# henreedev/audio-pathtracer

Measured on NVIDIA B200. Metric: bdpt_path_pairs_per_second, higher is better.
Workload: dtype f32 + u64 Q32.32

## Files before the change

### audio-pathtracer_b200/csrc/fs_api.cu

```cuda
#include "fs_internal.h"

#include <nvtx3/nvToolsExt.h>
#include <stdio.h>
#include <utility>
#include <stdlib.h>
#include <new>
#include <vector>

static thread_local std::string g_err;

#define CK(call)                                                                              \
    do {                                                                                      \
        cudaError_t e__ = (call);                                                             \
        if (e__ != cudaSuccess) return fail_cuda(ctx, e__, #call);                            \
    } while (0)

static int fail(fs_ctx* ctx, int code, const char* msg)
{
    (void)ctx;
    g_err = msg;
    return code;
}
static int fail_cuda(fs_ctx* ctx, cudaError_t e, const char* what)
{
// ... 17 lines not shown
};

extern "C" {

void fs_default_config(fs_config* c)
{
    memset(c, 0, sizeof(*c));
    c->n_bands = 8; c->n_bins = 1000; c->bin_ms = 1.0f; c->rr_prob = 0.9f;
    c->eps_offset = 1e-3f; c->eps_connect = 1e-3f; c->min_seg = 1e-2f; c->sound_speed = 343.0f;
    c->pdf_exponent = 0.1f; c->energy_clamp = 1.0f; c->energy_gain = 10.0f;
    static const float air[FS_MAX_BANDS] = {0.0001f, 0.0003f, 0.0006f, 0.0010f, 0.0017f, 0.0035f, 0.0050f, 0.0120f};
    for (int b = 0; b < FS_MAX_BANDS; ++b) c->air_absorption[b] = air[b];
    c->sample_rate = 48000; c->n_channels = 2; c->ir_threshold = 1e-6f; c->ir_lowpass = 0.25f;
    c->conv_block = 1024; c->conv_clamp = 1; c->conv_wet = 1.0f;
    c->max_batch_paths = 0; c->flags = 0; c->device = -1;
}

const char* fs_last_error(const fs_ctx* ctx) { (void)ctx; return g_err.c_str(); }

int fs_create(const fs_config* cfg, fs_ctx** out)
{
    if (!cfg || !out) return fail(nullptr, FS_ERR_INVALID, "fs_create: null argument");
    *out = nullptr;
    if (cfg->n_bands < 1 || cfg->n_bands > FS_MAX_BANDS) return fail(nullptr, FS_ERR_INVALID, "n_bands must be 1..8");
    if (cfg->n_bins < 1 || cfg->n_bins > (1u << 20)) return fail(nullptr, FS_ERR_INVALID, "n_bins out of range");
    if (!(cfg->bin_ms > 0.f) || !(cfg->sound_speed > 0.f)) return fail(nullptr, FS_ERR_INVALID, "bin_ms/sound_speed must be > 0");
    if (!(cfg->rr_prob > 0.f) || cfg->rr_prob > 1.0f) return fail(nullptr, FS_ERR_INVALID, "rr_prob must be in (0,1]");
    if (cfg->n_channels < 1 || cfg->n_channels > 8) return fail(nullptr, FS_ERR_INVALID, "n_channels must be 1..8");
    if (cfg->conv_block < 32 || cfg->conv_block > 2048 || (cfg->conv_block & (cfg->conv_block - 1)))
        return fail(nullptr, FS_ERR_INVALID, "conv_block must be a power of two in 32..2048");
    if (cfg->sample_rate < cfg->conv_block) return fail(nullptr, FS_ERR_INVALID, "sample_rate < conv_block");
    if ((uint32_t)((double)cfg->bin_ms * 1e-3 * cfg->sample_rate + 0.5) < 1u)
        return fail(nullptr, FS_ERR_INVALID, "bin_ms * sample_rate / 1000 must be at least one sample");
    if (!(cfg->ir_lowpass > 0.0f) || cfg->ir_lowpass > 1.0f) return fail(nullptr, FS_ERR_INVALID, "ir_lowpass must be in (0,1]");
    uint32_t ir_window = 32;
    if (cfg->ir_lowpass < 1.0f) {
        const double w = ceil(log(1e-12) / log(1.0 - (double)cfg->ir_lowpass));
        if (!(w <= 8192.0)) return fail(nullptr, FS_ERR_INVALID, "ir_lowpass too small (needs a warm-up window above 8192 samples)");
        ir_window = ((uint32_t)w + 31u) & ~31u;
        if (ir_window < 32u) ir_window = 32u;
    }
    int ndev = 0;
    cudaError_t e = cudaGetDeviceCount(&ndev);
    if (e != cudaSuccess || ndev == 0) {
        char buf[256];
        snprintf(buf, sizeof(buf), "no usable CUDA device (%s); this library has no CPU fallback",
                 e == cudaSuccess ? "device count 0" : cudaGetErrorString(e));
        return fail(nullptr, FS_ERR_CUDA, buf);
    }
    int dev = cfg->device;
    if (dev < 0) { if (cudaGetDevice(&dev) != cudaSuccess) dev = 0; }
    if (dev >= ndev) return fail(nullptr, FS_ERR_INVALID, "device ordinal out of range");
    fs_ctx* ctx = new (std::nothrow) fs_ctx();
    if (!ctx) return fail(nullptr, FS_ERR_NOMEM, "out of host memory");
    ctx->cfg = *cfg;
    if (ctx->cfg.max_batch_paths == 0) ctx->cfg.max_batch_paths = 1u << 21;
    ctx->device = dev;
    ctx->ir_window = ir_window;
    ctx->launches.store(0); ctx->conv_active.store(0);
    ctx->tune_refill = 4; ctx->tune_leaf_max = FS_LEAF_MAX; ctx->tune_tex = 2; ctx->tune_builder = 1; ctx->tune_wide = 1; ctx->tune_node_min = 14; ctx->tune_tri_min = 4; ctx->tune_collapse = 17 ; ctx->tune_l2pin_mb = 0xffffffffu ; ctx->tune_streams = 2;
    if (const char* e14 = getenv("FS_TUNE_STREAMS")) { int v = atoi(e14); if (v >= 1 && v <= FS_MAX_LANES) ctx->tune_streams = (uint32_t)v; } ctx->tune_tq = 2;
    ctx->tune_tq_node_min = 10; ctx->tune_tq_flush = 24;
    if (const char* e11 = getenv("FS_TUNE_TQ")) ctx->tune_tq = (uint32_t)atoi(e11);
    ctx->tune_mega = 2;
    if (const char* e15 = getenv("FS_TUNE_MEGA")) ctx->tune_mega = (uint32_t)atoi(e15);
    ctx->tune_mega_from = 0; ctx->tune_mega_lanes = 2;
    if (const char* e16 = getenv("FS_TUNE_MEGA_FROM")) ctx->tune_mega_from = (uint32_t)atoi(e16);
    if (const char* e17 = getenv("FS_TUNE_MEGA_LANES")) { int v = atoi(e17); if (v >= 1 && v <= FS_MAX_LANES) ctx->tune_mega_lanes = (uint32_t)v; }
    if (const char* e12 = getenv("FS_TUNE_TQ_NODE_MIN")) ctx->tune_tq_node_min = (uint32_t)atoi(e12);
    if (const char* e13 = getenv("FS_TUNE_TQ_FLUSH")) ctx->tune_tq_flush = (uint32_t)atoi(e13);
    if (ctx->tune_tq_flush < 1) ctx->tune_tq_flush = 1;
    if (ctx->tune_tq_flush > 32) ctx->tune_tq_flush = 32;
    if (const char* e10 = getenv("FS_TUNE_L2PIN")) ctx->tune_l2pin_mb = (uint32_t)atoi(e10);
    if (const char* e9 = getenv("FS_TUNE_COLLAPSE")) ctx->tune_collapse = (uint32_t)atoi(e9);
    if (const char* e7 = getenv("FS_TUNE_TRI_MIN")) ctx->tune_tri_min = (uint32_t)atoi(e7);
    if (const char* e6 = getenv("FS_TUNE_NODE_MIN")) ctx->tune_node_min = (uint32_t)atoi(e6);
    if (const char* e5 = getenv("FS_TUNE_WIDE")) ctx->tune_wide = (uint32_t)atoi(e5);
    ctx->tune_w8 = 0;
    if (const char* e18 = getenv("FS_TUNE_W8")) ctx->tune_w8 = (uint32_t)atoi(e18);
    if (const char* e4 = getenv("FS_TUNE_BUILDER")) ctx->tune_builder = (uint32_t)atoi(e4);
    if (const char* e3 = getenv("FS_TUNE_TEX")) ctx->tune_tex = (uint32_t)atoi(e3);
    if (const char* e1 = getenv("FS_TUNE_REFILL")) { int v = atoi(e1); if (v >= 1 && v <= 32) ctx->tune_refill = (uint32_t)v; }
    if (const char* e2 = getenv("FS_TUNE_LEAF_MAX")) { int v = atoi(e2); if (v >= 1 && v <= 8) ctx->tune_leaf_max = (uint32_t)v; }
    dev_guard g(dev);
    int rc = FS_OK;
    do {
        cudaDeviceProp prop;
        if ((e = cudaGetDeviceProperties(&prop, dev)) != cudaSuccess) { rc = fail_cuda(nullptr, e, "cudaGetDeviceProperties"); break; }
        if (prop.major < 10) {
            char buf[256];
            snprintf(buf, sizeof(buf), "device %d is sm_%d%d; this library is built for sm_100a only", dev, prop.major, prop.minor);
            rc = fail(nullptr, FS_ERR_CUDA, buf); break;
        }
        ctx->sm_count = prop.multiProcessorCount;
        if ((e = cudaStreamCreateWithFlags(&ctx->own_stream, cudaStreamNonBlocking)) != cudaSuccess) { rc = fail_cuda(nullptr, e, "cudaStreamCreate"); break; }
        ctx->stream = ctx->own_stream;
        if ((e = cudaEventCreate(&ctx->ev0)) != cudaSuccess || (e = cudaEventCreate(&ctx->ev1)) != cudaSuccess ||
            (e = cudaEventCreate(&ctx->ev_ir0)) != cudaSuccess || (e = cudaEventCreate(&ctx->ev_ir1)) != cudaSuccess) { rc = fail_cuda(nullptr, e, "cudaEventCreate"); break; }
        if ((e = cudaEventCreateWithFlags(&ctx->ev_fork, cudaEventDisableTiming)) != cudaSuccess) { rc = fail_cuda(nullptr, e, "cudaEventCreate"); break; }
        if ((e = cudaEventCreateWithFlags(&ctx->ev_overflow, cudaEventDisableTiming)) != cudaSuccess) { rc = fail_cuda(nullptr, e, "cudaEventCreate"); break; }
        if ((e = cudaEventCreate(&ctx->ev_c0)) != cudaSuccess || (e = cudaEventCreate(&ctx->ev_c1)) != cudaSuccess) { rc = fail_cuda(nullptr, e, "cudaEventCreate"); break; }
        if ((e = cudaMallocHost(&ctx->h_overflow, sizeof(uint32_t))) != cudaSuccess) { rc = fail_cuda(nullptr, e, "cudaMallocHost"); break; }
        *ctx->h_overflow = 0u;
        for (int l = 1; l < FS_MAX_LANES && e == cudaSuccess; ++l) {
            if ((e = cudaStreamCreateWithFlags(&ctx->lanes[l].stream, cudaStreamNonBlocking)) != cudaSuccess) break;
            e = cudaEventCreateWithFlags(&ctx->lanes[l].done, cudaEventDisableTiming);
        }
        if (e != cudaSuccess) { rc = fail_cuda(nullptr, e, "batch lanes"); break; }
        if ((e = cudaMalloc(&ctx->d_counters, sizeof(fs_dev_counters))) != cudaSuccess) { rc = fail_cuda(nullptr, e, "cudaMalloc counters"); break; }
        if ((e = cudaMemsetAsync(ctx->d_counters, 0, sizeof(fs_dev_counters), ctx->own_stream)) != cudaSuccess ||
            (e = cudaStreamSynchronize(ctx->own_stream)) != cudaSuccess) { rc = fail_cuda(nullptr, e, "cudaMemset"); break; }
        if ((e = cudaMalloc(&ctx->d_amp, sizeof(float) * cfg->n_bins)) != cudaSuccess) { rc = fail_cuda(nullptr, e, "cudaMalloc amp"); break; }
        if ((e = cudaMalloc(&ctx->d_energy, sizeof(float) * cfg->n_bins)) != cudaSuccess) { rc = fail_cuda(nullptr, e, "cudaMalloc energy"); break; }
        if ((e = fs_conv_setup(ctx)) != cudaSuccess) { rc = fail_cuda(nullptr, e, "fs_conv_setup"); break; }
    } while (0);
    if (rc != FS_OK) { fs_destroy(ctx); return rc; }
    *out = ctx;
    return FS_OK;
}

void fs_destroy(fs_ctx* ctx)
{
    if (!ctx) return;
    dev_guard g(ctx->device);
    cudaDeviceSynchronize();
    fs_conv_teardown(ctx);
    cudaFree(ctx->d_carriers); cudaFree(ctx->d_amp_bands); cudaFree(ctx->d_amp_all);
    cudaFree(ctx->lis_rec); cudaFree(ctx->lis_end);
    for (int l = 0; l < FS_MAX_LANES; ++l) {
        fs_wave_free(&ctx->lanes[l].wb);
        if (l && ctx->lanes[l].stream) cudaStreamDestroy(ctx->lanes[l].stream);
        if (ctx->lanes[l].done) cudaEventDestroy(ctx->lanes[l].done);
    }
    if (ctx->ev_fork) cudaEventDestroy(ctx->ev_fork);
    if (ctx->ev_overflow) cudaEventDestroy(ctx->ev_overflow);
    if (ctx->ev_c0) cudaEventDestroy(ctx->ev_c0);
    if (ctx->ev_c1) cudaEventDestroy(ctx->ev_c1);
    if (ctx->h_overflow) cudaFreeHost(ctx->h_overflow);
    cudaFree(ctx->d_bsdf_tab); cudaFree(ctx->d_lobes);
    fs_bvh_free(&ctx->bvh);
    cudaFree(ctx->d_verts); cudaFree(ctx->d_tri_mat); cudaFree(ctx->d_refl_over_pi);
    cudaFree(ctx->d_hist); cudaFree(ctx->d_counters); cudaFree(ctx->d_src_pos); cudaFree(ctx->d_dbg);
    cudaFree(ctx->d_amp); cudaFree(ctx->d_energy);
    for (cudaEvent_t e : ctx->kev) cudaEventDestroy(e);
    for (cudaEvent_t e : ctx->tev) cudaEventDestroy(e);
    if (ctx->ev0) cudaEventDestroy(ctx->ev0);
    if (ctx->ev1) cudaEventDestroy(ctx->ev1);
    if (ctx->ev_ir0) cudaEventDestroy(ctx->ev_ir0);
    if (ctx->ev_ir1) cudaEventDestroy(ctx->ev_ir1);
    if (ctx->own_stream) cudaStreamDestroy(ctx->own_stream);
    delete ctx;
}

static void apply_l2_policy(fs_ctx* ctx);

static int check_overflow(fs_ctx* ctx, bool wait)
{
    if (!ctx->overflow_pending) return FS_OK;
    if (wait) { CK(cudaEventSynchronize(ctx->ev_overflow)); }
    else if (cudaEventQuery(ctx->ev_overflow) != cudaSuccess) { (void)cudaGetLastError(); return FS_OK; }
    ctx->overflow_pending = false;
    if (*ctx->h_overflow) {
        *ctx->h_overflow = 0u;
        return fail(ctx, FS_ERR_OVERFLOW, "BVH traversal stack overflow in the last trace (tree deeper than FS_STACK_SIZE): its histogram is incomplete");
    }
    return FS_OK;
// ... 95 lines not shown
int fs_scene_set_materials_ex(fs_ctx* ctx, const float* absorption, const float* transmission, const float* scattering,
                              const float* thickness_cm, uint32_t n_materials, uint32_t n_bands)
{
    int rc = fs_scene_set_materials(ctx, absorption, n_materials, n_bands);
    if (rc != FS_OK) return rc;
    const size_t n = (size_t)n_materials * n_bands;
    for (int which = 0; which < 2; ++which) {
        const float* v = which ? scattering : transmission;
        if (!v) continue;
        for (size_t i = 0; i < n; ++i)
            if (!(v[i] >= 0.0f && v[i] <= 1.0f)) return fail(ctx, FS_ERR_INVALID, which ? "scattering must be in [0,1]" : "transmission must be in [0,1]");
    }
    if (thickness_cm)
        for (uint32_t m = 0; m < n_materials; ++m)
            if (!(thickness_cm[m] >= 0.0f)) return fail(ctx, FS_ERR_INVALID, "thickness must be >= 0");
    ctx->mat_transmission.assign(transmission ? transmission : nullptr, transmission ? transmission + n : nullptr);
    ctx->mat_scattering.assign(scattering ? scattering : nullptr, scattering ? scattering + n : nullptr);
    ctx->mat_thickness_cm.assign(thickness_cm ? thickness_cm : nullptr, thickness_cm ? thickness_cm + n_materials : nullptr);
    ctx->committed = false;
    return FS_OK;
}

static int build_material_model(fs_ctx* ctx)
{
    const uint32_t M = ctx->n_mats, B = ctx->cfg.n_bands;
    std::vector<float> tab((size_t)3 * M * B, 0.0f);
    std::vector<float4> lobes(M);
    const float* tr = ctx->mat_transmission.empty() ? nullptr : ctx->mat_transmission.data();
    const float* sc = ctx->mat_scattering.empty() ? nullptr : ctx->mat_scattering.data();
    const float* th = ctx->mat_thickness_cm.empty() ? nullptr : ctx->mat_thickness_cm.data();
    for (uint32_t m = 0; m < M; ++m) {
        float sum_r = 0.0f, sum_t = 0.0f, sum_s = 0.0f;
        const float thick = th ? th[m] : 2.5f;
        const float ex = thick / 2.5f;
        for (uint32_t b = 0; b < B; ++b) {
            const float a = ctx->mat_absorption[(size_t)m * B + b];
            const float refl = 1.0f - a;
            float tau = tr ? tr[(size_t)m * B + b] : 0.0f;
            if (refl + tau > 1.0f) tau = 1.0f - refl;
            const float sig = sc ? sc[(size_t)m * B + b] : 1.0f;
            float tau_eff = 0.0f;
            if (tau > 0.0f) tau_eff = (ex == 1.0f) ? tau : fs_pow(tau, ex);
            tab[((size_t)0 * M + m) * B + b] = (refl * sig) / FS_PI;
            tab[((size_t)1 * M + m) * B + b] = refl * (1.0f - sig);
            tab[((size_t)2 * M + m) * B + b] = tau_eff;
            sum_r += refl; sum_t += tau; sum_s += sig;
        }
        const float mr = sum_r / (float)B, mt = sum_t / (float)B, ms = sum_s / (float)B;
        const float tot = mr + mt;
        const float t1 = (tot > 0.0f) ? mt / tot : 0.0f;
        const float ps = (1.0f - t1) * (1.0f - ms);
        const float t2 = t1 + ps;
        const float pd = 1.0f - t2;
        lobes[m] = make_float4(t1, t2, ps, pd);
    }
    cudaFree(ctx->d_bsdf_tab); cudaFree(ctx->d_lobes); ctx->d_bsdf_tab = nullptr; ctx->d_lobes = nullptr;
    CK(cudaMalloc(&ctx->d_bsdf_tab, sizeof(float) * tab.size()));
    CK(cudaMalloc(&ctx->d_lobes, sizeof(float4) * lobes.size()));
    CK(cudaMemcpyAsync(ctx->d_bsdf_tab, tab.data(), sizeof(float) * tab.size(), cudaMemcpyHostToDevice, ctx->stream));
    CK(cudaMemcpyAsync(ctx->d_lobes, lobes.data(), sizeof(float4) * lobes.size(), cudaMemcpyHostToDevice, ctx->stream));
    CK(cudaStreamSynchronize(ctx->stream));
    return FS_OK;
}

int fs_scene_commit(fs_ctx* ctx)
{
    if (!ctx) return FS_ERR_INVALID;
    if (!ctx->tris_set || !ctx->mats_set) return fail(ctx, FS_ERR_STATE, "fs_scene_commit: set triangles and materials first");
    nvtx_range nv("fs_scene_commit (BVH build)");
    dev_guard g(ctx->device);
    if (ctx->n_tris) {
        std::vector<uint32_t> m(ctx->n_tris);
        CK(cudaMemcpyAsync(m.data(), ctx->d_tri_mat, sizeof(uint32_t) * ctx->n_tris, cudaMemcpyDeviceToHost, ctx->stream));
        CK(cudaStreamSynchronize(ctx->stream));
        for (uint64_t i = 0; i < ctx->n_tris; ++i)
            if (m[i] >= ctx->n_mats) return fail(ctx, FS_ERR_INVALID, "triangle material id out of range");
    }
    if (ctx->cfg.flags & FS_FLAG_MATERIAL_MODEL) {
        int rc = build_material_model(ctx);
        if (rc) return rc;
    }
    uint64_t bvh_launches = 0;
    CK(fs_bvh_build(ctx->stream, ctx->d_verts, ctx->d_tri_mat, ctx->n_tris, &ctx->bvh, &bvh_launches,
                    ctx->tune_leaf_max, ctx->tune_builder, ctx->tune_collapse | (ctx->tune_w8 ? 4u : 0u)));
    CK(cudaStreamSynchronize(ctx->stream));
    ctx->launches.fetch_add(bvh_launches);
    ctx->stats.bvh_nodes = ctx->bvh.n_inner;
    if (getenv("FS_VERBOSE")) fprintf(stderr, "[frequensee] BVH: %u triangles, %u BVH2 nodes, %u reachable 4-wide nodes (%.1f MB)\n",
                                      ctx->bvh.n_tris, ctx->bvh.n_inner, ctx->bvh.n_wide, ctx->bvh.n_wide * 64.0 / 1e6);
    if (getenv("FS_VERBOSE") && ctx->bvh.w8nodes) fprintf(stderr, "[frequensee] BVH: %u 8-wide compressed nodes (%.1f MB)\n", ctx->bvh.n_w8, ctx->bvh.n_w8 * 80.0 / 1e6);
    ctx->stats.bvh_max_leaf = ctx->bvh.max_leaf;
    apply_l2_policy(ctx);
    ctx->committed = true;
    ctx->verts_dirty = false;
    return FS_OK;
}

static bool host_is_pinned(const void* p);

int fs_scene_update_vertices(fs_ctx* ctx, const float* verts, uint64_t first_tri, uint64_t n_tris)
{
    if (!ctx) return FS_ERR_INVALID;
    if (!ctx->tris_set) return fail(ctx, FS_ERR_STATE, "fs_scene_update_vertices: call fs_scene_set_triangles first");
    if (n_tris && !verts) return fail(ctx, FS_ERR_INVALID, "fs_scene_update_vertices: null array");
    if (first_tri > ctx->n_tris || n_tris > ctx->n_tris - first_tri)
        return fail(ctx, FS_ERR_INVALID, "fs_scene_update_vertices: triangle range outside the scene");
    for (uint64_t i = 0; i < n_tris * 9; ++i)
        if (!(verts[i] == verts[i]) || fabsf(verts[i]) > 1e18f) return fail(ctx, FS_ERR_INVALID, "non-finite vertex");
    if (!n_tris) return FS_OK;
    dev_guard g(ctx->device);
    CK(cudaMemcpyAsync(ctx->d_verts + first_tri * 9, verts, sizeof(float) * 9 * n_tris, cudaMemcpyHostToDevice, ctx->stream));
    if (host_is_pinned(verts)) CK(cudaStreamSynchronize(ctx->stream));
    if (ctx->committed) ctx->verts_dirty = true;
    return FS_OK;
}

int fs_scene_refit(fs_ctx* ctx, float* cost_ratio_out)
{
    if (!ctx) return FS_ERR_INVALID;
    if (!ctx->committed) return fail(ctx, FS_ERR_STATE, "fs_scene_refit: call fs_scene_commit first");
    nvtx_range nv("fs_scene_refit");
    if (ctx->tune_w8) {
        int rc = fs_scene_commit(ctx);
        if (rc == FS_OK && cost_ratio_out) *cost_ratio_out = 1.0f;
        return rc;
    }
    dev_guard g(ctx->device);
    uint64_t launches = 0;
    float ratio = 1.0f;
    CK(fs_bvh_refit(ctx->stream, ctx->d_verts, &ctx->bvh, &launches, &ratio));
    ctx->launches.fetch_add(launches);
    ctx->verts_dirty = false;
    if (cost_ratio_out) *cost_ratio_out = ratio;
    return FS_OK;
}

static void fill_params(fs_ctx* ctx, fs_trace_params* tp, const float lis[3], uint64_t n_paths, uint32_t max_depth,
                        uint64_t seed)
{
    const fs_config& c = ctx->cfg;
    memset(tp, 0, sizeof(*tp));
    tp->bv.nodes_tex = (ctx->tune_tex && ctx->bvh.nodes_tex) ? (unsigned long long)ctx->bvh.nodes_tex : 0ull;
    tp->bv.tris_tex = (ctx->tune_tex && ctx->bvh.tris_tex) ? (unsigned long long)ctx->bvh.tris_tex : 0ull;
    tp->bv.wnodes = ctx->tune_wide ? ctx->bvh.wnodes : nullptr;
    tp->bv.wnodes_tex = (ctx->tune_tex && ctx->bvh.wnodes_tex) ? (unsigned long long)ctx->bvh.wnodes_tex : 0ull;
    const bool w8 = ctx->tune_w8 && ctx->tune_wide && ctx->bvh.w8nodes;
    tp->bv.w8nodes = w8 ? ctx->bvh.w8nodes : nullptr; tp->bv.tris8 = w8 ? ctx->bvh.tris8 : nullptr; tp->bv.tri8_map = w8 ? ctx->bvh.tri8_map : nullptr;
    tp->bv.w8_magic = 0x47000000u;
    for (int a = 0; a < 3; ++a) { tp->bv.qbase[a] = ctx->bvh.qbase[a]; tp->bv.qscale[a] = ctx->bvh.qscale[a]; }
    tp->bv.nodes = ctx->bvh.nodes; tp->bv.tris = ctx->bvh.tris; tp->bv.tri_orig = ctx->bvh.tri_orig;
    tp->bv.tri_mat = ctx->bvh.tri_mat; tp->bv.tri_nm = ctx->bvh.tri_nm; tp->bv.n_tris = ctx->bvh.n_tris; tp->bv.n_inner = ctx->bvh.n_inner;
    tp->top = ctx->bvh.top_nodes; tp->n_top = ctx->bvh.n_top;
    const bool model = (c.flags & FS_FLAG_MATERIAL_MODEL) && ctx->d_lobes;
    tp->refl_over_pi = model ? ctx->d_bsdf_tab : ctx->d_refl_over_pi; tp->n_mats = ctx->n_mats;
    tp->lobes = model ? ctx->d_lobes : nullptr;
    tp->ep.min_seg = c.min_seg; tp->ep.pdf_exponent = c.pdf_exponent; tp->ep.n_bands = c.n_bands;
    for (int b = 0; b < FS_MAX_BANDS; ++b) tp->ep.air[b] = c.air_absorption[b];
    tp->n_bins = c.n_bins; tp->bin_ms = c.bin_ms; tp->rr_prob = c.rr_prob; tp->eps_offset = c.eps_offset;
    tp->eps_connect = c.eps_connect; tp->sound_speed = c.sound_speed; tp->energy_clamp = c.energy_clamp;
    tp->energy_gain = c.energy_gain; tp->max_depth = max_depth;
    tp->seed_lo = (uint32_t)seed; tp->seed_hi = (uint32_t)(seed >> 32);
    tp->n_paths = n_paths;
    tp->src_pos = ctx->d_src_pos;
    if (lis) { tp->lis[0] = lis[0]; tp->lis[1] = lis[1]; tp->lis[2] = lis[2]; }
    tp->flags = c.flags;
}

// ... 676 lines not shown
```

### audio-pathtracer_b200/csrc/fs_bvh.cuh

```cuda
#pragma once

#include "fs_math.cuh"

#define FS_STACK_SIZE 64
#define FS_LEAF_MAX 4
#define FS_TOP_FLAG 0x40000000

#if defined(FS_TRAVERSAL_GUARD)
#define FS_GUARD_DECL uint32_t guard_ = 0;
#define FS_GUARD_STEP if (++guard_ > 4000000u) { *overflow = 2u; node = SENTINEL; sp = 0; break; }
#else
#define FS_GUARD_DECL
#define FS_GUARD_STEP
#endif

struct fs_bvh_view {
    unsigned long long nodes_tex;
    unsigned long long tris_tex;
    unsigned long long wnodes_tex;
    const uint4* wnodes;
    const uint4* w8nodes;
    const float4* tris8;
    const uint32_t* tri8_map;
    uint32_t w8_magic;
    float qbase[3], qscale[3];
    const float4* nodes;
    const float4* tris;
    const uint32_t* tri_orig;
    const uint32_t* tri_mat;
    const float4* tri_nm;
    uint32_t n_tris;
    uint32_t n_inner;
};

struct fs_visit_counters { uint32_t nodes, tris; };

#if defined(__CUDACC__)

__device__ __forceinline__ float4 fs_ldg4(const float4* p)
{
    float4 r;
    asm volatile("ld.global.nc.v4.f32 {%0, %1, %2, %3}, [%4];"
                 : "=f"(r.x), "=f"(r.y), "=f"(r.z), "=f"(r.w) : "l"(p));
    return r;
}

__device__ __forceinline__ void fs_ldg8(const float4* p, float4& a, float4& b)
{
    asm volatile("ld.global.nc.v8.f32 {%0, %1, %2, %3, %4, %5, %6, %7}, [%8];"
                 : "=f"(a.x), "=f"(a.y), "=f"(a.z), "=f"(a.w), "=f"(b.x), "=f"(b.y), "=f"(b.z), "=f"(b.w)
                 : "l"(p));
}

struct fs_ray_prep {
    fs_vec3 o, d;
    float idx, idy, idz, oodx, oody, oodz;
};

__device__ __forceinline__ fs_ray_prep fs_prep_ray(fs_vec3 o, fs_vec3 d)
{
    fs_ray_prep r;
    r.o = o; r.d = d;
    float dx = (fabsf(d.x) > 1e-30f) ? d.x : ((d.x < 0.0f) ? -1e-30f : 1e-30f);
    float dy = (fabsf(d.y) > 1e-30f) ? d.y : ((d.y < 0.0f) ? -1e-30f : 1e-30f);
    float dz = (fabsf(d.z) > 1e-30f) ? d.z : ((d.z < 0.0f) ? -1e-30f : 1e-30f);
    r.idx = 1.0f / dx; r.idy = 1.0f / dy; r.idz = 1.0f / dz;
    r.oodx = o.x * r.idx; r.oody = o.y * r.idy; r.oodz = o.z * r.idz;
    return r;
}

__device__ __forceinline__ void fs_slab2(const fs_ray_prep& r, float4 n0, float4 n1, float4 n2,
                                         float tmax, bool& h0, bool& h1, float& t0n, float& t1n)
{
    float c0lox = fmaf(n0.x, r.idx, -r.oodx), c0hix = fmaf(n0.y, r.idx, -r.oodx);
    float c0loy = fmaf(n0.z, r.idy, -r.oody), c0hiy = fmaf(n0.w, r.idy, -r.oody);
    float c0loz = fmaf(n2.x, r.idz, -r.oodz), c0hiz = fmaf(n2.y, r.idz, -r.oodz);
    float c1lox = fmaf(n1.x, r.idx, -r.oodx), c1hix = fmaf(n1.y, r.idx, -r.oodx);
    float c1loy = fmaf(n1.z, r.idy, -r.oody), c1hiy = fmaf(n1.w, r.idy, -r.oody);
    float c1loz = fmaf(n2.z, r.idz, -r.oodz), c1hiz = fmaf(n2.w, r.idz, -r.oodz);
    float c0min = fmaxf(fmaxf(fminf(c0lox, c0hix), fminf(c0loy, c0hiy)), fmaxf(fminf(c0loz, c0hiz), 0.0f));
    float c0max = fminf(fminf(fmaxf(c0lox, c0hix), fmaxf(c0loy, c0hiy)), fminf(fmaxf(c0loz, c0hiz), tmax));
    float c1min = fmaxf(fmaxf(fminf(c1lox, c1hix), fminf(c1loy, c1hiy)), fmaxf(fminf(c1loz, c1hiz), 0.0f));
    float c1max = fminf(fminf(fmaxf(c1lox, c1hix), fmaxf(c1loy, c1hiy)), fminf(fmaxf(c1loz, c1hiz), tmax));
    h0 = c0min <= c0max;
    h1 = c1min <= c1max;
    t0n = c0min; t1n = c1min;
}

// ... 117 lines not shown
```

### audio-pathtracer_b200/csrc/fs_bvh_build.cu

```cuda
#include "fs_internal.h"
#include <vector>
#include <utility>
#include <stdlib.h>

namespace {

__device__ __forceinline__ uint32_t f2ord(float f)
{
    uint32_t u = __float_as_uint(f);
    return (u & 0x80000000u) ? ~u : (u | 0x80000000u);
}
__host__ __device__ __forceinline__ float ord2f(uint32_t u)
{
    u = (u & 0x80000000u) ? (u & 0x7fffffffu) : ~u;
#if defined(__CUDA_ARCH__)
    return __uint_as_float(u);
#else
    float f; memcpy(&f, &u, 4); return f;
#endif
}

__global__ void k_init_bounds(uint32_t* bounds)
{
    if (threadIdx.x < 3) bounds[threadIdx.x] = 0xffffffffu;
// ... 469 lines not shown
    cbox c[4];
    int k = 2;
    load_children(nodes, (int)i, c[0], c[1]);
    if (collapse) {
        while (k < 4) {
            int pick = -1; float best = -1.0f;
            for (int j = 0; j < k; ++j)
                if (c[j].ref >= 0) { const float a = cbox_area(c[j]); if (a > best) { best = a; pick = j; } }
            if (pick < 0) break;
            const int r = c[pick].ref;
            load_children(nodes, r, c[pick], c[k]);
            ++k;
        }
    } else {
        const int r0 = c[0].ref, r1 = c[1].ref;
        if (r1 >= 0) { load_children(nodes, r1, c[1], c[k]); ++k; }
        if (r0 >= 0) { load_children(nodes, r0, c[0], c[k]); ++k; }
    }
    for (int j = 0; j < 4; ++j) {
        wnodes[(size_t)i * 4 + j] = (j < k) ? quant_box(c[j].lx, c[j].hx, c[j].ly, c[j].hy, c[j].lz, c[j].hz, c[j].ref, grid) : EMPTY;
        wsrc[(size_t)i * 4 + j] = (j < k) ? c[j].src : -1;
    }
}

__device__ __forceinline__ bool wide_is_inner(uint32_t ref) { return (int)ref >= 0 && ref != 0x7fffffffu; }

__global__ void k_wide_count(const uint4* __restrict__ src, const int* __restrict__ frontier, uint32_t nf, uint32_t* __restrict__ cnt)
{
    const uint32_t t = blockIdx.x * blockDim.x + threadIdx.x;
    if (t >= nf) return;
    const uint4* p = src + (size_t)frontier[t] * 4;
    uint32_t c = 0;
    for (int j = 0; j < 4; ++j) c += wide_is_inner(p[j].w) ? 1u : 0u;
    cnt[t] = c;
}

__global__ void k_wide_place(const uint4* __restrict__ src, uint4* __restrict__ dst, const int* __restrict__ src_prov,
                             int* __restrict__ dst_prov, const int* __restrict__ frontier, uint32_t nf,
                             const uint32_t* __restrict__ off, uint32_t level_base, int* __restrict__ next_frontier)
{
    const uint32_t t = blockIdx.x * blockDim.x + threadIdx.x;
    if (t >= nf) return;
    const uint4* p = src + (size_t)frontier[t] * 4;
    uint4* q = dst + (size_t)(level_base + t) * 4;
    uint32_t o = off[t];
    for (int j = 0; j < 4; ++j) {
        uint4 u = p[j];
        if (wide_is_inner(u.w)) { next_frontier[o] = (int)u.w; u.w = level_base + nf + o; ++o; }
        q[j] = u;
        dst_prov[(size_t)(level_base + t) * 4 + j] = src_prov[(size_t)frontier[t] * 4 + j];
    }
}

#define W8_EMPTY 0x7fffffff
__device__ __forceinline__ uint32_t q8_lo(float v, float p, float inv)
{
    const float q = floorf((v - p) * inv - 0.001953125f);
    return (uint32_t)fminf(fmaxf(q, 0.0f), 255.0f);
}
__device__ __forceinline__ uint32_t q8_hi(float v, float p, float inv)
{
    const float q = ceilf((v - p) * inv + 0.001953125f);
    return (uint32_t)fminf(fmaxf(q, 0.0f), 255.0f);
}
__device__ __forceinline__ int q8_exponent(float ext)
{
    int k = -60;
    if (ext > 1e-18f) { (void)frexpf(ext / 254.0f, &k); }
    k = k < -60 ? -60 : (k > 60 ? 60 : k);
    return k + 127;
}

__global__ void k_w8_parents(uint32_t n_inner, const float4* __restrict__ nodes, int* __restrict__ parent, uint32_t* __restrict__ need)
{
    const uint32_t i = blockIdx.x * blockDim.x + threadIdx.x;
    if (i >= n_inner) return;
    const float4 n3 = nodes[(size_t)i * 4 + 3];
    const int c0 = __float_as_int(n3.x), c1 = __float_as_int(n3.y);
    need[i] = (c0 >= 0 ? 1u : 0u) + (c1 >= 0 ? 1u : 0u);
    if (c0 >= 0) parent[c0] = (int)i;
    if (c1 >= 0) parent[c1] = (int)i;
    if (i == 0) parent[0] = -1;
}
template <int W>
__device__ __forceinline__ float wide_t(const float* T, int ref, int j) { return ref >= 0 ? __ldcg(T + (size_t)ref * W + (j - 1)) : 0.0f; }
__device__ __forceinline__ float w8_t(const float* T, int ref, int j) { return wide_t<8>(T, ref, j); }
template <int W>
__global__ void k_wide_dp(uint32_t n_inner, const float4* __restrict__ nodes, const int* __restrict__ parent,
                        const uint32_t* __restrict__ need, uint32_t* __restrict__ arrive, float* T)
{
    const uint32_t i = blockIdx.x * blockDim.x + threadIdx.x;
    if (i >= n_inner || need[i] != 0u) return;
    int n = (int)i;
    for (;;) {
        cbox a, b;
        load_children(nodes, n, a, b);
        float ta[W], tb[W], t[W];
        for (int j = 1; j <= W; ++j) { ta[j - 1] = wide_t<W>(T, a.ref, j); tb[j - 1] = wide_t<W>(T, b.ref, j); }
        cbox u;
        u.lx = fminf(a.lx, b.lx); u.hx = fmaxf(a.hx, b.hx); u.ly = fminf(a.ly, b.ly); u.hy = fmaxf(a.hy, b.hy);
        u.lz = fminf(a.lz, b.lz); u.hz = fmaxf(a.hz, b.hz);
        float best = 3.0e38f;
        for (int x = 1; x <= W - 1; ++x) best = fminf(best, ta[x - 1] + tb[W - 1 - x]);
        t[0] = cbox_area(u) + best;
        for (int j = 2; j <= W; ++j) {
            float m = t[j - 2];
            for (int x = 1; x < j; ++x) m = fminf(m, ta[x - 1] + tb[j - x - 1]);
            t[j - 1] = m;
        }
        for (int j = 0; j < W; ++j) T[(size_t)n * W + j] = t[j];
        __threadfence();
        const int p = parent[n];
        if (p < 0) break;
        if (atomicAdd(arrive + p, 1u) + 1u < need[p]) break;
        n = p;
    }
}

template <int W>
__device__ __forceinline__ int dp_cut(const float4* __restrict__ nodes, const float* __restrict__ T, int i, cbox* c)
{
    cbox st[W]; int sb[W]; int sp = 0, k = 0;
    {
        cbox l, r;
        load_children(nodes, i, l, r);
        float best = 3.0e38f; int ba = 1;
        for (int x = 1; x <= W - 1; ++x) { const float v = wide_t<W>(T, l.ref, x) + wide_t<W>(T, r.ref, W - x); if (v < best) { best = v; ba = x; } }
        st[0] = l; sb[0] = ba; st[1] = r; sb[1] = W - ba; sp = 2;
    }
    while (sp) {
        --sp;
        const cbox m = st[sp]; const int j = sb[sp];
        if (m.ref < 0 || j == 1) { c[k++] = m; continue; }
        cbox x, y;
        load_children(nodes, m.ref, x, y);
        float best = wide_t<W>(T, m.ref, 1); int ba = 0;
        for (int q = 1; q < j; ++q) { const float v = wide_t<W>(T, x.ref, q) + wide_t<W>(T, y.ref, j - q); if (v < best) { best = v; ba = q; } }
        if (!ba) { c[k++] = m; continue; }
        st[sp] = x; sb[sp] = ba; st[sp + 1] = y; sb[sp + 1] = j - ba; sp += 2;
    }
    return k;
}

__global__ void k_emit4_dp(uint32_t n_inner, const float4* __restrict__ nodes, const float* __restrict__ T, const float* __restrict__ grid,
                           uint4* __restrict__ wnodes, int* __restrict__ wsrc)
{
    const uint32_t i = blockIdx.x * blockDim.x + threadIdx.x;
    if (i >= n_inner) return;
    const uint4 EMPTY = make_uint4(0x0000ffffu, 0x0000ffffu, 0x0000ffffu, 0x7fffffffu);
    cbox c[4];
    const int k = dp_cut<4>(nodes, T, (int)i, c);
    for (int j = 0; j < 4; ++j) {
        wnodes[(size_t)i * 4 + j] = (j < k) ? quant_box(c[j].lx, c[j].hx, c[j].ly, c[j].hy, c[j].lz, c[j].hz, c[j].ref, grid) : EMPTY;
        wsrc[(size_t)i * 4 + j] = (j < k) ? c[j].src : -1;
    }
}

__global__ void k_emit8(uint32_t n_inner, const float4* __restrict__ nodes, const float* __restrict__ T, uint4* __restrict__ w8tmp,
                        int* __restrict__ w8ref)
{
    const uint32_t i = blockIdx.x * blockDim.x + threadIdx.x;
    if (i >= n_inner) return;
    cbox c[8];
    int k = 2;
    if (T) {
        k = dp_cut<8>(nodes, T, (int)i, c);
    } else {
        load_children(nodes, (int)i, c[0], c[1]);
        while (k < 8) {
            int pick = -1; float best = -1.0f;
            for (int j = 0; j < k; ++j)
                if (c[j].ref >= 0) { const float a = cbox_area(c[j]); if (a > best) { best = a; pick = j; } }
            if (pick < 0) break;
            const int r = c[pick].ref;
            load_children(nodes, r, c[pick], c[k]);
            ++k;
        }
    }
    float lx = c[0].lx, hx = c[0].hx, ly = c[0].ly, hy = c[0].hy, lz = c[0].lz, hz = c[0].hz;
    for (int j = 1; j < k; ++j) {
        lx = fminf(lx, c[j].lx); hx = fmaxf(hx, c[j].hx); ly = fminf(ly, c[j].ly); hy = fmaxf(hy, c[j].hy);
        lz = fminf(lz, c[j].lz); hz = fmaxf(hz, c[j].hz);
    }
    if (!(hx < 1e29f) || !(lx > -1e29f) || !(hy < 1e29f) || !(hz < 1e29f)) {
        hx = fminf(hx, 1e29f); hy = fminf(hy, 1e29f); hz = fminf(hz, 1e29f);
    }
    const float mx = 0.5f * (lx + hx), my = 0.5f * (ly + hy), mz = 0.5f * (lz + hz);
    int slot_of[8], child_in[8];
    for (int j = 0; j < 8; ++j) { slot_of[j] = -1; child_in[j] = -1; }
    for (int it = 0; it < k; ++it) {
        float best = -3.0e38f; int bc = -1, bs = -1;
        for (int j = 0; j < k; ++j) {
            if (slot_of[j] >= 0) continue;
            const float dx = 0.5f * (c[j].lx + c[j].hx) - mx, dy = 0.5f * (c[j].ly + c[j].hy) - my, dz = 0.5f * (c[j].lz + c[j].hz) - mz;
            for (int s = 0; s < 8; ++s) {
                if (child_in[s] >= 0) continue;
                const float cost = ((s & 1) ? dx : -dx) + ((s & 2) ? dy : -dy) + ((s & 4) ? dz : -dz);
                if (cost > best) { best = cost; bc = j; bs = s; }
            }
        }
        slot_of[bc] = bs; child_in[bs] = bc;
    }
    const int ebx = q8_exponent(hx - lx), eby = q8_exponent(hy - ly), ebz = q8_exponent(hz - lz);
    const float ix = __uint_as_float((uint32_t)(254 - ebx) << 23), iy = __uint_as_float((uint32_t)(254 - eby) << 23),
                iz = __uint_as_float((uint32_t)(254 - ebz) << 23);
    uint32_t q[12];
    for (int w = 0; w < 12; ++w) q[w] = 0u;
    uint32_t imask = 0, lmask = 0;
    int refs[8];
    for (int s = 0; s < 8; ++s) {
        const int j = child_in[s];
        uint32_t b[6];
        if (j < 0) { b[0] = b[1] = b[2] = 255u; b[3] = b[4] = b[5] = 0u; refs[s] = W8_EMPTY; }
        else {
            b[0] = q8_lo(c[j].lx, lx, ix); b[1] = q8_lo(c[j].ly, ly, iy); b[2] = q8_lo(c[j].lz, lz, iz);
            b[3] = q8_hi(c[j].hx, lx, ix); b[4] = q8_hi(c[j].hy, ly, iy); b[5] = q8_hi(c[j].hz, lz, iz);
            refs[s] = c[j].ref;
            if (c[j].ref >= 0) imask |= 1u << s; else lmask |= 1u << s;
        }
        for (int a = 0; a < 6; ++a) q[a * 2 + (s >> 2)] |= b[a] << (8 * (s & 3));
    }
    uint4* o = w8tmp + (size_t)i * 5;
    o[0] = make_uint4(__float_as_uint(lx), __float_as_uint(ly), __float_as_uint(lz), ((uint32_t)ebx << 23) | imask | (lmask << 8));
    o[1] = make_uint4((uint32_t)eby << 23, (uint32_t)ebz << 23, 0u, 0u);
    o[2] = make_uint4(q[0], q[1], q[2], q[3]);
    o[3] = make_uint4(q[4], q[5], q[6], q[7]);
    o[4] = make_uint4(q[8], q[9], q[10], q[11]);
    for (int s = 0; s < 8; ++s) w8ref[(size_t)i * 8 + s] = refs[s];
}

__global__ void k_w8_count(const uint4* __restrict__ w8tmp, const int* __restrict__ frontier, uint32_t nf,
                           uint32_t* __restrict__ cnt_in, uint32_t* __restrict__ cnt_leaf)
{
    const uint32_t t = blockIdx.x * blockDim.x + threadIdx.x;
    if (t >= nf) return;
    const uint32_t w = w8tmp[(size_t)frontier[t] * 5].w;
    cnt_in[t] = (uint32_t)__popc(w & 0xffu);
    cnt_leaf[t] = (uint32_t)__popc((w >> 8) & 0xffu);
}

__global__ void k_w8_place(const uint4* __restrict__ w8tmp, const int* __restrict__ w8ref, uint4* __restrict__ dst,
                           const int* __restrict__ frontier, uint32_t nf, const uint32_t* __restrict__ off_in,
                           const uint32_t* __restrict__ off_leaf, uint32_t level_base, uint32_t tri_level_base,
                           int* __restrict__ next_frontier, const float4* __restrict__ tris, float4* __restrict__ tris8,
                           uint32_t* __restrict__ tri8_map)
{
    const uint32_t t = blockIdx.x * blockDim.x + threadIdx.x;
    if (t >= nf) return;
    const int src = frontier[t];
// ... 502 lines not shown
    BCHECK(cudaStreamSynchronize(st));
    {
        uint64_t acc = 0;
        for (int bin = 4095; bin >= 0; --bin) {
            acc += h_hist[bin];
            if (acc * 10 >= n_slots) { thr = ord2f((uint32_t)bin << 20); break; }
        }
    }
    prev = cost0;
    for (it = 0; it < iters; ++it) {
        struct { double cost; uint32_t moved; } h;
        BCHECK(cudaMemsetAsync(lock, 0, 8ull * n_inner, st));
        BCHECK(cudaMemsetAsync(misc, 0, 16, st));
        k_w8_parents<<<gi, TPB, 0, st>>>(n_inner, nodes, parent, need);
        k_ri_search<<<gs, TPB, 0, st>>>(n_inner, nodes, parent, thr, 1e-5f, mv_gain, mv_dst);
        k_ri_lock<<<gs, TPB, 0, st>>>(n_inner, parent, mv_gain, mv_dst, lock);
        BCHECK(cudaMemcpyAsync(backup, nodes, sizeof(float4) * 4ull * n_inner, cudaMemcpyDeviceToDevice, st));
        k_ri_apply<<<gs, TPB, 0, st>>>(n_inner, parent, mv_gain, mv_dst, lock, nodes, (uint32_t*)(misc + 8));
        BCHECK(cudaMemsetAsync(arrive, 0, 4ull * n_inner, st));
        k_w8_parents<<<gi, TPB, 0, st>>>(n_inner, nodes, parent, need);
        k_refit_nodes<<<gi, TPB, 0, st>>>(n_inner, d_verts, tri_orig, parent, need, arrive, nodes, ubox);
        k_sah_cost<<<gi, TPB, 0, st>>>(n_inner, nodes, (double*)misc);
        *launches += 7;
        BCHECK(cudaMemcpyAsync(&h, misc, sizeof(h), cudaMemcpyDeviceToHost, st));
        BCHECK(cudaStreamSynchronize(st));
        BCHECK(cudaGetLastError());
        if (h.moved == 0) break;
        if (h.cost > prev) {
            BCHECK(cudaMemcpyAsync(nodes, backup, sizeof(float4) * 4ull * n_inner, cudaMemcpyDeviceToDevice, st));
            BCHECK(cudaStreamSynchronize(st));
            break;
        }
        total_moves += h.moved;
        const bool small = prev - h.cost < 1e-4 * prev;
        prev = h.cost;
        if (small) { ++it; break; }
    }
    if (getenv("FS_VERBOSE"))
        fprintf(stderr, "[frequensee] reinsertion: %d iterations, %u moves, surface-area cost %.6g -> %.6g (%.2f %%)\n", it,
                total_moves, cost0, prev, cost0 > 0.0 ? 100.0 * (prev - cost0) / cost0 : 0.0);
fail:
    cudaFree(parent); cudaFree(need); cudaFree(arrive); cudaFree(ubox); cudaFree(backup); cudaFree(lock);
    cudaFree(mv_gain); cudaFree(mv_dst); cudaFree(hist); cudaFree(misc);
    return err;
}

static cudaError_t wide_compact(cudaStream_t st, uint32_t n_inner, const uint4* sparse, const int* sparse_prov, uint4** dense_out,
                                int** dense_prov_out, uint32_t* n_wide_out, uint64_t* launches)
{
    cudaError_t err = cudaSuccess;
    int* fr[2] = {nullptr, nullptr};
    uint32_t *cnt = nullptr, *off = nullptr, *tile_sums = nullptr, *total = nullptr;
    uint4* dense = nullptr;
    int* dense_prov = nullptr;
    const int TPB = 256;
    uint32_t nf = 1, base = 0;
    int pp = 0;
    const int zero = 0;
    BCHECK(cudaMalloc(&fr[0], 4ull * n_inner)); BCHECK(cudaMalloc(&fr[1], 4ull * n_inner));
    BCHECK(cudaMalloc(&cnt, 4ull * n_inner)); BCHECK(cudaMalloc(&off, 4ull * n_inner));
    BCHECK(cudaMalloc(&tile_sums, 4ull * ((n_inner + SCAN_TILE - 1) / SCAN_TILE + 2)));
    BCHECK(cudaMalloc(&total, 4));
    BCHECK(cudaMalloc(&dense, sizeof(uint4) * 4ull * n_inner));
    BCHECK(cudaMalloc(&dense_prov, sizeof(int) * 4ull * n_inner));
    BCHECK(cudaMemcpyAsync(fr[0], &zero, 4, cudaMemcpyHostToDevice, st));
    while (nf) {
        const uint32_t g = (nf + TPB - 1) / TPB;
        uint32_t next = 0;
        k_wide_count<<<g, TPB, 0, st>>>(sparse, fr[pp], nf, cnt); ++*launches;
        scan_u32(st, cnt, off, nf, tile_sums, total, launches);
        k_wide_place<<<g, TPB, 0, st>>>(sparse, dense, sparse_prov, dense_prov, fr[pp], nf, off, base, fr[pp ^ 1]); ++*launches;
        BCHECK(cudaMemcpyAsync(&next, total, 4, cudaMemcpyDeviceToHost, st));
        BCHECK(cudaStreamSynchronize(st));
        base += nf; nf = next; pp ^= 1;
        if (base + nf > n_inner) { err = cudaErrorUnknown; goto fail; }
    }
    BCHECK(cudaGetLastError());
    *dense_out = dense; dense = nullptr; *dense_prov_out = dense_prov; dense_prov = nullptr; *n_wide_out = base;
fail:
    cudaFree(fr[0]); cudaFree(fr[1]); cudaFree(cnt); cudaFree(off); cudaFree(tile_sums); cudaFree(total); cudaFree(dense); cudaFree(dense_prov);
    return err;
}

static cudaError_t w8_build(cudaStream_t st, uint32_t n, uint32_t n_inner, const float4* nodes, const float4* tris,
                            fs_bvh_device* out, uint64_t* launches, bool dp)
{
    cudaError_t err = cudaSuccess;
    float* T = nullptr; int* parent = nullptr; uint32_t *need = nullptr, *arrive = nullptr;
    uint4 *tmp = nullptr, *dense = nullptr, *fit = nullptr;
    int *ref = nullptr, *fr[2] = {nullptr, nullptr};
    uint32_t *cnt_in = nullptr, *cnt_leaf = nullptr, *off_in = nullptr, *off_leaf = nullptr, *tile_sums = nullptr, *total = nullptr;
    float4* tris8 = nullptr; uint32_t* map = nullptr;
    const int TPB = 256;
    uint32_t nf = 1, base = 0, tri_base = 0;
    int pp = 0;
    const int zero = 0;
    BCHECK(cudaMalloc(&tmp, sizeof(uint4) * 5ull * n_inner));
    BCHECK(cudaMalloc(&ref, 4ull * 8 * n_inner));
    BCHECK(cudaMalloc(&dense, sizeof(uint4) * 5ull * n_inner));
    BCHECK(cudaMalloc(&fr[0], 4ull * n_inner)); BCHECK(cudaMalloc(&fr[1], 4ull * n_inner));
    BCHECK(cudaMalloc(&cnt_in, 4ull * n_inner)); BCHECK(cudaMalloc(&cnt_leaf, 4ull * n_inner));
    BCHECK(cudaMalloc(&off_in, 4ull * n_inner)); BCHECK(cudaMalloc(&off_leaf, 4ull * n_inner));
    BCHECK(cudaMalloc(&tile_sums, 4ull * ((n_inner + SCAN_TILE - 1) / SCAN_TILE + 2)));
    BCHECK(cudaMalloc(&total, 8));
    BCHECK(cudaMalloc(&tris8, sizeof(float4) * 4ull * n));
    BCHECK(cudaMalloc(&map, 4ull * n));
    if (dp) {
        BCHECK(cudaMalloc(&T, sizeof(float) * 8ull * n_inner));
        BCHECK(cudaMalloc(&parent, 4ull * n_inner)); BCHECK(cudaMalloc(&need, 4ull * n_inner)); BCHECK(cudaMalloc(&arrive, 4ull * n_inner));
        BCHECK(cudaMemsetAsync(arrive, 0, 4ull * n_inner, st));
        k_w8_parents<<<(n_inner + TPB - 1) / TPB, TPB, 0, st>>>(n_inner, nodes, parent, need);
        k_wide_dp<8><<<(n_inner + TPB - 1) / TPB, TPB, 0, st>>>(n_inner, nodes, parent, need, arrive, T);
        *launches += 2;
    }
    k_emit8<<<(n_inner + TPB - 1) / TPB, TPB, 0, st>>>(n_inner, nodes, T, tmp, ref); ++*launches;
    BCHECK(cudaMemcpyAsync(fr[0], &zero, 4, cudaMemcpyHostToDevice, st));
    while (nf) {
        const uint32_t g = (nf + TPB - 1) / TPB;
        uint32_t next[2] = {0, 0};
        k_w8_count<<<g, TPB, 0, st>>>(tmp, fr[pp], nf, cnt_in, cnt_leaf); ++*launches;
        scan_u32(st, cnt_in, off_in, nf, tile_sums, total, launches);
        scan_u32(st, cnt_leaf, off_leaf, nf, tile_sums, total + 1, launches);
        k_w8_place<<<g, TPB, 0, st>>>(tmp, ref, dense, fr[pp], nf, off_in, off_leaf, base, tri_base, fr[pp ^ 1], tris, tris8, map);
        ++*launches;
        BCHECK(cudaMemcpyAsync(next, total, 8, cudaMemcpyDeviceToHost, st));
        BCHECK(cudaStreamSynchronize(st));
        base += nf; nf = next[0]; tri_base += next[1]; pp ^= 1;
        if ((uint64_t)base + nf > n_inner || tri_base > n) { err = cudaErrorUnknown; goto fail; }
    }
    BCHECK(cudaGetLastError());
    if (tri_base != n) { err = cudaErrorUnknown; goto fail; }
    BCHECK(cudaMalloc(&fit, sizeof(uint4) * 5ull * base));
    BCHECK(cudaMemcpyAsync(fit, dense, sizeof(uint4) * 5ull * base, cudaMemcpyDeviceToDevice, st));
    BCHECK(cudaStreamSynchronize(st));
    out->w8nodes = fit; fit = nullptr; out->n_w8 = base;
    out->tris8 = tris8; tris8 = nullptr; out->tri8_map = map; map = nullptr;
fail:
    cudaFree(T); cudaFree(parent); cudaFree(need); cudaFree(arrive);
    cudaFree(tmp); cudaFree(ref); cudaFree(dense); cudaFree(fit); cudaFree(fr[0]); cudaFree(fr[1]); cudaFree(cnt_in); cudaFree(cnt_leaf);
    cudaFree(off_in); cudaFree(off_leaf); cudaFree(tile_sums); cudaFree(total); cudaFree(tris8); cudaFree(map);
    return err;
}

cudaError_t fs_bvh_build(cudaStream_t st, const float* d_verts, const uint32_t* d_mats, uint64_t T64,
                         fs_bvh_device* out, uint64_t* launches, uint32_t leaf_max_u, uint32_t builder, uint32_t collapse_u)
{
    const int leaf_max = (int)(leaf_max_u < 1 ? 1 : (leaf_max_u > 8 ? 8 : leaf_max_u));
    const int collapse = (int)collapse_u;
    cudaError_t err = cudaSuccess;
    const uint32_t n = (uint32_t)T64;
    fs_bvh_free(out);
    out->n_tris = n;
    if (n == 0) return cudaSuccess;
    const uint32_t n_inner = n > 1 ? n - 1 : 1;
    const uint32_t n_blocks_sort = (n + SORT_TILE - 1) / SORT_TILE;
    float4 *tlo = nullptr, *thi = nullptr, *bb_lo = nullptr, *bb_hi = nullptr;
    uint64_t *keys0 = nullptr, *keys1 = nullptr;
    uint32_t *vals0 = nullptr, *vals1 = nullptr, *block_hist = nullptr, *misc = nullptr, *arrive = nullptr;
    float* grid = nullptr;
    int2 *children = nullptr, *ranges = nullptr;
    int *parent = nullptr, *queue = nullptr;
    const int TPB = 256;
    const uint32_t gb = (n + TPB - 1) / TPB;

    BCHECK(cudaMalloc(&tlo, sizeof(float4) * n));
    BCHECK(cudaMalloc(&thi, sizeof(float4) * n));
    BCHECK(cudaMalloc(&bb_lo, sizeof(float4) * (2ull * n)));
    BCHECK(cudaMalloc(&bb_hi, sizeof(float4) * (2ull * n)));
    BCHECK(cudaMalloc(&keys0, 8ull * n));
    BCHECK(cudaMalloc(&keys1, 8ull * n));
    BCHECK(cudaMalloc(&vals0, 4ull * n));
    BCHECK(cudaMalloc(&vals1, 4ull * n));
    BCHECK(cudaMalloc(&block_hist, 4ull * 256 * n_blocks_sort));
    BCHECK(cudaMalloc(&misc, 4 * 16));
    BCHECK(cudaMalloc(&arrive, 4ull * n_inner));
    BCHECK(cudaMalloc(&children, sizeof(int2) * n_inner));
    BCHECK(cudaMalloc(&ranges, sizeof(int2) * n_inner));
    BCHECK(cudaMalloc(&parent, 4ull * 2 * n));
    BCHECK(cudaMalloc(&queue, 4ull * FS_TOP_CAP));
    BCHECK(cudaMalloc(&out->nodes, sizeof(float4) * 4ull * n_inner));
    BCHECK(cudaMalloc(&out->wnodes, sizeof(uint4) * 4ull * n_inner));
    BCHECK(cudaMalloc(&out->wsrc, sizeof(int) * 4ull * n_inner));
    BCHECK(cudaMalloc(&grid, sizeof(float) * 8));
    BCHECK(cudaMalloc(&out->tris, sizeof(float4) * 4ull * n));
    BCHECK(cudaMalloc(&out->tri_orig, 4ull * n));
    BCHECK(cudaMalloc(&out->tri_mat, 4ull * n));
    BCHECK(cudaMalloc(&out->tri_nm, sizeof(float4) * (size_t)n));
    BCHECK(cudaMalloc(&out->top_nodes, sizeof(float4) * 4ull * FS_TOP_CAP));
    out->n_inner = n_inner;

    BCHECK(cudaMemsetAsync(misc, 0, 4 * 16, st));
    BCHECK(cudaMemsetAsync(arrive, 0, 4ull * n_inner, st));
    k_init_bounds<<<1, 32, 0, st>>>(misc); ++*launches;
    k_tri_bounds<<<gb, TPB, 0, st>>>(d_verts, n, tlo, thi, misc, misc + 6); ++*launches;
    k_morton<<<gb, TPB, 0, st>>>(tlo, thi, n, misc, keys0, vals0); ++*launches;
    {
        uint64_t *ki = keys0, *ko = keys1;
        uint32_t *vi = vals0, *vo = vals1;
        for (int pass = 0; pass < 8; ++pass) {
            int shift = pass * 8;
            k_sort_hist<<<n_blocks_sort, SORT_THREADS, 0, st>>>(ki, n, shift, block_hist, n_blocks_sort);
            k_sort_scan<<<1, 1024, 0, st>>>(block_hist, 256u * n_blocks_sort);
            k_sort_scatter<<<n_blocks_sort, SORT_THREADS, 0, st>>>(ki, vi, ko, vo, n, shift, block_hist, n_blocks_sort);
            *launches += 3;
            uint64_t* tk = ki; ki = ko; ko = tk;
            uint32_t* tv = vi; vi = vo; vo = tv;
        }
    }
    k_pack<<<gb, TPB, 0, st>>>(d_verts, d_mats, vals0, n, tlo, thi, out->tris, out->tri_orig, out->tri_mat, out->tri_nm, bb_lo, bb_hi);
    ++*launches;
    if (n == 1) {
        k_emit_single<<<1, 1, 0, st>>>(bb_lo, bb_hi, out->nodes); ++*launches;
        out->max_leaf = 1;
    } else if (builder == 1 && n >= 3) {
        int cand[4] = {5, 10, 24, 64}, n_cand = 4;
        if (const char* e = getenv("FS_TUNE_PLOC_R")) { int v = atoi(e); if (v >= 1 && v <= 256) { cand[0] = v; n_cand = 1; } }
        if (n < 4096) n_cand = 1;
        double best_cost = 0.0; int best = -1;
        float4* alt = nullptr; double* d_cost = nullptr;
        float* cT4 = nullptr; int* cpar = nullptr; uint32_t *cneed = nullptr, *carr = nullptr;
        if (n_cand > 1) { BCHECK(cudaMalloc(&alt, sizeof(float4) * 4ull * n_inner)); BCHECK(cudaMalloc(&d_cost, 8)); }
        for (int ci = 0; ci < n_cand; ++ci) {
            float4* dst = (n_cand > 1) ? alt : out->nodes;
            BCHECK(ploc_build(st, n, bb_lo, bb_hi, dst, launches, cand[ci]));
            if (n_cand == 1) break;
            double h_cost = 0.0;
            BCHECK(cudaMemsetAsync(d_cost, 0, 8, st));
            k_sah_cost<<<(n_inner + TPB - 1) / TPB, TPB, 0, st>>>(n_inner, dst, d_cost); ++*launches;
            BCHECK(cudaMemcpyAsync(&h_cost, d_cost, 8, cudaMemcpyDeviceToHost, st));
            BCHECK(cudaStreamSynchronize(st));
            if (getenv("FS_VERBOSE")) fprintf(stderr, "[frequensee] PLOC radius %d: surface-area cost %.6g\n", cand[ci], h_cost);
            if (collapse & 16) {
                if (!cT4) {
                    BCHECK(cudaMalloc(&cT4, sizeof(float) * 4ull * n_inner)); BCHECK(cudaMalloc(&cpar, 4ull * n_inner));
                    BCHECK(cudaMalloc(&cneed, 4ull * n_inner)); BCHECK(cudaMalloc(&carr, 4ull * n_inner));
                }
                float root_cost = 0.f;
                BCHECK(cudaMemsetAsync(carr, 0, 4ull * n_inner, st));
                k_w8_parents<<<(n_inner + TPB - 1) / TPB, TPB, 0, st>>>(n_inner, dst, cpar, cneed);
                k_wide_dp<4><<<(n_inner + TPB - 1) / TPB, TPB, 0, st>>>(n_inner, dst, cpar, cneed, carr, cT4);
                *launches += 2;
                BCHECK(cudaMemcpyAsync(&root_cost, cT4, 4, cudaMemcpyDeviceToHost, st));
                BCHECK(cudaStreamSynchronize(st));
                if (getenv("FS_VERBOSE")) fprintf(stderr, "[frequensee] PLOC radius %d: summed area of the 4-wide nodes %.6g\n", cand[ci], (double)root_cost);
                h_cost = (double)root_cost;
            }
            if (best < 0 || h_cost < best_cost) {
                best = ci; best_cost = h_cost;
                BCHECK(cudaMemcpyAsync(out->nodes, alt, sizeof(float4) * 4ull * n_inner, cudaMemcpyDeviceToDevice, st));
            }
        }
        if (alt) { cudaStreamSynchronize(st); cudaFree(alt); cudaFree(d_cost); }
        cudaFree(cT4); cudaFree(cpar); cudaFree(cneed); cudaFree(carr);
        out->max_leaf = 1;
        {
            int sweeps = 0;
            if (const char* e = getenv("FS_TUNE_ROTATE")) { int v = atoi(e); if (v >= 0 && v <= 64) sweeps = v; }
            if (sweeps && n >= 4096) {
                uint32_t n_rot = 0;
                BCHECK(bvh2_rotate(st, n_inner, out->nodes, sweeps, launches, &n_rot));
                if (getenv("FS_VERBOSE")) {
                    double* d_c = nullptr; double h_c = 0.0;
                    if (cudaMalloc(&d_c, 8) == cudaSuccess) {
                        cudaMemsetAsync(d_c, 0, 8, st);
                        k_sah_cost<<<(n_inner + TPB - 1) / TPB, TPB, 0, st>>>(n_inner, out->nodes, d_c);
                        cudaMemcpyAsync(&h_c, d_c, 8, cudaMemcpyDeviceToHost, st); cudaStreamSynchronize(st); cudaFree(d_c);
                    }
                    fprintf(stderr, "[frequensee] %d rotation sweeps: %u rotations, surface-area cost %.6g\n", sweeps, n_rot, h_c);
                }
            }
        }
        {
            int iters = FS_REINSERT_ITERS;
            if (const char* e = getenv("FS_TUNE_REINSERT")) { int v = atoi(e); if (v >= 0 && v <= 256) iters = v; }
            if (iters && n >= 4096) BCHECK(bvh2_reinsert(st, n_inner, d_verts, out->tri_orig, out->nodes, iters, launches));
        }
    } else {
        k_karras<<<gb, TPB, 0, st>>>(keys0, (int)n, children, ranges, parent); ++*launches;
        k_refit<<<gb, TPB, 0, st>>>((int)n, children, parent, bb_lo, bb_hi, arrive); ++*launches;
        k_emit<<<gb, TPB, 0, st>>>((int)n, children, ranges, bb_lo, bb_hi, out->nodes, leaf_max); ++*launches;
        k_leaf_stats<<<gb, TPB, 0, st>>>((int)n, ranges, misc + 8, leaf_max); ++*launches;
    }
    k_quant_grid<<<1, 32, 0, st>>>(out->nodes, grid); ++*launches;
    if ((collapse & 16) && n >= 3) {
        float* T4 = nullptr; int* par = nullptr; uint32_t *need = nullptr, *arr = nullptr;
        cudaError_t e4 = cudaSuccess;
        if ((e4 = cudaMalloc(&T4, sizeof(float) * 4ull * n_inner)) == cudaSuccess && (e4 = cudaMalloc(&par, 4ull * n_inner)) == cudaSuccess &&
            (e4 = cudaMalloc(&need, 4ull * n_inner)) == cudaSuccess && (e4 = cudaMalloc(&arr, 4ull * n_inner)) == cudaSuccess &&
            (e4 = cudaMemsetAsync(arr, 0, 4ull * n_inner, st)) == cudaSuccess) {
            k_w8_parents<<<(n_inner + TPB - 1) / TPB, TPB, 0, st>>>(n_inner, out->nodes, par, need);
            k_wide_dp<4><<<(n_inner + TPB - 1) / TPB, TPB, 0, st>>>(n_inner, out->nodes, par, need, arr, T4);
            k_emit4_dp<<<(n_inner + TPB - 1) / TPB, TPB, 0, st>>>(n_inner, out->nodes, T4, grid, out->wnodes, out->wsrc);
            *launches += 3;
            e4 = cudaStreamSynchronize(st);
        }
        cudaFree(T4); cudaFree(par); cudaFree(need); cudaFree(arr);
        BCHECK(e4);
    } else {
        k_emit4<<<(n_inner + TPB - 1) / TPB, TPB, 0, st>>>(n_inner, out->nodes, grid, out->wnodes, out->wsrc, collapse & 1); ++*launches;
    }
    out->n_wide = n_inner;
    if (!(collapse & 2)) {
        uint4* dense = nullptr; int* dense_prov = nullptr; uint32_t n_wide = 0;
        BCHECK(wide_compact(st, n_inner, out->wnodes, out->wsrc, &dense, &dense_prov, &n_wide, launches));
        cudaFree(out->wnodes); out->wnodes = dense; out->n_wide = n_wide;
        cudaFree(out->wsrc); out->wsrc = dense_prov;
    }
    {
        cudaResourceDesc rd; memset(&rd, 0, sizeof(rd));
        rd.resType = cudaResourceTypeLinear;
        rd.res.linear.devPtr = out->nodes;
        rd.res.linear.desc = cudaCreateChannelDesc<float4>();
        rd.res.linear.sizeInBytes = sizeof(float4) * 4ull * n_inner;
        cudaTextureDesc td; memset(&td, 0, sizeof(td));
        td.readMode = cudaReadModeElementType;
        if (cudaCreateTextureObject(&out->nodes_tex, &rd, &td, nullptr) != cudaSuccess) { out->nodes_tex = 0; (void)cudaGetLastError(); }
        rd.res.linear.devPtr = out->tris;
        rd.res.linear.sizeInBytes = sizeof(float4) * 4ull * n;
        if (cudaCreateTextureObject(&out->tris_tex, &rd, &td, nullptr) != cudaSuccess) { out->tris_tex = 0; (void)cudaGetLastError(); }
        rd.res.linear.devPtr = out->wnodes;
        rd.res.linear.desc = cudaCreateChannelDesc<uint4>();
        rd.res.linear.sizeInBytes = sizeof(uint4) * 4ull * out->n_wide;
        if (cudaCreateTextureObject(&out->wnodes_tex, &rd, &td, nullptr) != cudaSuccess) { out->wnodes_tex = 0; (void)cudaGetLastError(); }
    }
    k_top_treelet<<<1, 32, 0, st>>>(out->nodes, n_inner, FS_TOP_CAP, out->top_nodes, misc + 7, queue); ++*launches;
    BCHECK(cudaGetLastError());
    if (builder == 1 && n >= 3 && out->max_leaf == 1 && (collapse & 4)) BCHECK(w8_build(st, n, n_inner, out->nodes, out->tris, out, launches, !(collapse & 8)));
    {
        uint32_t h[16];
        BCHECK(cudaMemcpyAsync(h, misc, sizeof(h), cudaMemcpyDeviceToHost, st));
        BCHECK(cudaStreamSynchronize(st));
        out->n_top = h[7];
        if (n > 1 && !(builder == 1 && n >= 3)) out->max_leaf = h[8] ? h[8] : 1;
        out->extent = ord2f(h[6]);
        float hg[6];
        BCHECK(cudaMemcpy(hg, grid, sizeof(hg), cudaMemcpyDeviceToHost));
        for (int a = 0; a < 3; ++a) { out->qbase[a] = hg[a]; out->qscale[a] = hg[3 + a]; }
    }
fail:
    cudaFree(tlo); cudaFree(thi); cudaFree(bb_lo); cudaFree(bb_hi); cudaFree(keys0); cudaFree(keys1);
    cudaFree(vals0); cudaFree(vals1); cudaFree(block_hist); cudaFree(misc); cudaFree(arrive);
    cudaFree(children); cudaFree(ranges); cudaFree(parent); cudaFree(queue); cudaFree(grid);
    if (err != cudaSuccess) fs_bvh_free(out);
    return err;
}

void fs_bvh_free(fs_bvh_device* b)
{
    if (b->nodes_tex) cudaDestroyTextureObject(b->nodes_tex);
    if (b->tris_tex) cudaDestroyTextureObject(b->tris_tex);
    if (b->wnodes_tex) cudaDestroyTextureObject(b->wnodes_tex);
    cudaFree(b->w8nodes); cudaFree(b->tris8); cudaFree(b->tri8_map);
    cudaFree(b->nodes); cudaFree(b->wnodes); cudaFree(b->tris); cudaFree(b->tri_orig); cudaFree(b->tri_mat); cudaFree(b->tri_nm); cudaFree(b->top_nodes);
    cudaFree(b->wsrc);
    cudaFree(b->rf.parent); cudaFree(b->rf.need); cudaFree(b->rf.arrive); cudaFree(b->rf.ubox); cudaFree(b->rf.queue); cudaFree(b->rf.misc);
    memset(b, 0, sizeof(*b));
}

cudaError_t fs_bvh_refit(cudaStream_t st, const float* d_verts, fs_bvh_device* b, uint64_t* launches, float* cost_ratio)
{
    cudaError_t err = cudaSuccess;
    const uint32_t n = b->n_tris, n_inner = b->n_inner;
    const int TPB = 256;
    fs_bvh_device::refit_scratch& r = b->rf;
    struct { double cost[2]; float grid[8]; uint32_t n_top; } h;
    if (cost_ratio) *cost_ratio = 1.0f;
    if (n == 0) return cudaSuccess;
    if (!r.misc) {
        BCHECK(cudaMalloc(&r.parent, 4ull * n_inner));
        BCHECK(cudaMalloc(&r.need, 4ull * n_inner));
        BCHECK(cudaMalloc(&r.arrive, 4ull * n_inner));
        BCHECK(cudaMalloc(&r.ubox, sizeof(float4) * 2ull * n_inner));
        BCHECK(cudaMalloc(&r.queue, 4ull * FS_TOP_CAP));
        BCHECK(cudaMalloc(&r.misc, sizeof(h)));
        BCHECK(cudaMemsetAsync(r.parent, 0xff, 4ull * n_inner, st));
        BCHECK(cudaMemsetAsync(r.misc, 0, sizeof(h), st));
        k_w8_parents<<<(n_inner + TPB - 1) / TPB, TPB, 0, st>>>(n_inner, b->nodes, r.parent, r.need);
        k_sah_cost<<<(n_inner + TPB - 1) / TPB, TPB, 0, st>>>(n_inner, b->nodes, (double*)r.misc);
        *launches += 2;
        BCHECK(cudaMemcpyAsync(&r.cost0, r.misc, sizeof(double), cudaMemcpyDeviceToHost, st));
    }
    BCHECK(cudaMemsetAsync(r.arrive, 0, 4ull * n_inner, st));
    BCHECK(cudaMemsetAsync((double*)r.misc + 1, 0, sizeof(double), st));
    k_refit_tris<<<(n + TPB - 1) / TPB, TPB, 0, st>>>(n, d_verts, b->tri_orig, b->tri_mat, b->tris, b->tri_nm);
    if (n == 1) k_refit_single<<<1, 1, 0, st>>>(d_verts, b->tri_orig, b->nodes);
    else k_refit_nodes<<<(n_inner + TPB - 1) / TPB, TPB, 0, st>>>(n_inner, d_verts, b->tri_orig, r.parent, r.need, r.arrive, b->nodes, r.ubox);
    k_sah_cost<<<(n_inner + TPB - 1) / TPB, TPB, 0, st>>>(n_inner, b->nodes, (double*)r.misc + 1);
    {
        float* d_grid = (float*)((char*)r.misc + offsetof(decltype(h), grid));
        k_quant_grid<<<1, 32, 0, st>>>(b->nodes, d_grid);
        const uint32_t n_slots = 4u * b->n_wide;
        k_requant4<<<(n_slots + TPB - 1) / TPB, TPB, 0, st>>>(n_slots, b->nodes, b->wsrc, d_grid, b->wnodes);
        k_top_treelet<<<1, 32, 0, st>>>(b->nodes, n_inner, FS_TOP_CAP, b->top_nodes,
                                        (uint32_t*)((char*)r.misc + offsetof(decltype(h), n_top)), r.queue);
    }
    *launches += 6;
    BCHECK(cudaGetLastError());
    BCHECK(cudaMemcpyAsync(&h, r.misc, sizeof(h), cudaMemcpyDeviceToHost, st));
    BCHECK(cudaStreamSynchronize(st));
    for (int a = 0; a < 3; ++a) { b->qbase[a] = h.grid[a]; b->qscale[a] = h.grid[3 + a]; }
    b->n_top = h.n_top;
    if (cost_ratio) *cost_ratio = r.cost0 > 0.0 ? (float)(h.cost[1] / r.cost0) : 1.0f;
fail:
    return err;
}
```

### audio-pathtracer_b200/csrc/fs_internal.h

```cpp
#pragma once

#include <cuda_runtime.h>
#include <stdint.h>
#include <string.h>
#include <string>
#include <atomic>
#include <mutex>
#include <vector>

#include "../../include/frequensee.h"
#include "fs_math.cuh"
#include "fs_bvh.cuh"

#define FS_TOP_CAP 1024

struct fs_bvh_device {
    float4* nodes;
    float4* tris;
    uint32_t* tri_orig;
    uint32_t* tri_mat;
    float4* tri_nm;
    float4* top_nodes;
    cudaTextureObject_t nodes_tex, tris_tex, wnodes_tex;
    uint4* wnodes;
    float qbase[3], qscale[3];
    uint32_t n_tris, n_inner, n_top, max_leaf;
    uint32_t n_wide;
    uint4* w8nodes;
    float4* tris8;
    uint32_t* tri8_map;
    uint32_t n_w8;
    float extent;
    int* wsrc;
    struct refit_scratch {
        int* parent;
        uint32_t* need;
        uint32_t* arrive;
        float4* ubox;
        int* queue;
        void* misc;
        double cost0;
    } rf;
};

cudaError_t fs_bvh_build(cudaStream_t st, const float* d_verts, const uint32_t* d_mats, uint64_t n_tris,
                         fs_bvh_device* out, uint64_t* launches, uint32_t leaf_max, uint32_t builder ,
                         uint32_t collapse );
void fs_bvh_free(fs_bvh_device* b);
cudaError_t fs_bvh_refit(cudaStream_t st, const float* d_verts, fs_bvh_device* b, uint64_t* launches, float* cost_ratio);

struct fs_dev_counters {
    unsigned long long ext_rays, shadow_rays, connected, node_visits, tri_tests;
    unsigned long long shadow_node_visits, shadow_tri_tests;
    uint32_t overflow, max_steps;
    uint32_t steps_hist[16];
};

struct fs_trace_params {
    fs_bvh_view bv;
    const float4* top;
    uint32_t n_top;
    const float* refl_over_pi;
    const float4* lobes;
    uint32_t n_mats;
    fs_eval_params ep;
    uint32_t n_bins;
    float bin_ms, rr_prob, eps_offset, eps_connect, sound_speed, energy_clamp, energy_gain;
    uint32_t max_depth;
    uint32_t seed_lo, seed_hi;
    uint64_t n_paths;
    uint64_t g_first;
    uint32_t batch;
    uint32_t cap;
    const float* src_pos;
    float lis[3];
    uint32_t flags;
    uint32_t lis_mode;
    float4* lis_rec;
    float4* lis_end;
};

struct fs_wave_buffers {
    float4* st_pos[2];
    float4* st_nrm[2];
    float4* rec;
    float4* end_pos;
    float2* hit;
    uint32_t* conn_queue;
    float* conn_len;
    uint32_t* q_count;
    uint32_t* q_cursor;
    uint32_t cap, depth_cap;
    float4* npos;
    float4* nnrm;
    float4 *all_o, *all_d;
    uint32_t* all_conn;
    uint64_t all_cap;
    float4 *log_o, *log_d; uint32_t* log_flag; void* pq; uint32_t log_cap, pq_epoch;
};

struct fs_conv_source {
    bool active;
    float2* fdl;
    float2* H[2];
    float* prev;
    float* ir;
    int pub, pending;
    cudaEvent_t h_ready[2];
    uint32_t head;
};

#define FS_MEGA_MIN_BATCH (1u << 17)
#define FS_MAX_LANES 4
#define FS_MAX_SOURCES 4096
#define FS_PTR_TABLE 64
struct fs_ptr_table { void* p[FS_PTR_TABLE]; void* q[FS_PTR_TABLE]; };

struct fs_lane { cudaStream_t stream; fs_wave_buffers wb; cudaEvent_t done; };

struct fs_ctx {
    fs_config cfg;
    int device;
    cudaStream_t own_stream, stream;
    cudaStream_t conv_stream;
    float* d_verts; uint32_t* d_tri_mat; uint64_t n_tris;
    float* d_refl_over_pi; uint32_t n_mats;
    float* d_bsdf_tab; float4* d_lobes;
    std::vector<float> mat_absorption;
    std::vector<float> mat_transmission, mat_scattering, mat_thickness_cm;
    bool mats_set, tris_set, committed;
    bool verts_dirty;
    fs_bvh_device bvh;
    fs_lane lanes[FS_MAX_LANES];
    cudaEvent_t ev_fork; uint32_t tune_streams;
    float4 *lis_rec, *lis_end; uint64_t lis_cache_n; uint32_t lis_cache_depth;
    unsigned long long* d_hist; uint32_t hist_sources;
    uint32_t hist_cur_sources;
    uint64_t hist_n_paths;
    fs_dev_counters* d_counters;
    uint32_t* h_overflow; cudaEvent_t ev_overflow; bool overflow_pending;
    float* d_src_pos; uint32_t src_cap;
    fs_path_dbg* d_dbg; uint64_t dbg_cap;
    fs_stats stats;
    std::atomic<uint64_t> launches;
    std::atomic<int> conv_active;
    cudaEvent_t ev0, ev1, ev_ir0, ev_ir1; bool timed, ir_timed;
    std::vector<cudaEvent_t> kev; size_t kev_used;
    std::vector<cudaEvent_t> tev; size_t tev_used;
    int sm_count;
    int occ[16];
    uint32_t tune_refill, tune_leaf_max, tune_tex, tune_builder, tune_wide, tune_node_min, tune_tri_min, tune_collapse, tune_l2pin_mb, tune_tq, tune_tq_node_min, tune_tq_flush, tune_mega, tune_mega_from, tune_mega_lanes, cur_lanes, tune_w8;
    float* d_energy;
    float* d_amp;
    float* d_amp_all; uint32_t amp_all_cap;
    float* d_carriers; float* d_amp_bands; uint64_t carrier_seed;
    float2* d_twiddle;
    uint32_t fft_n, n_part, n_freq, ir_window;
    std::vector<fs_conv_source*> conv;
    float *d_conv_in, *d_conv_out; size_t conv_io_cap;
    float *h_pin_in, *h_pin_out;
    cudaEvent_t ev_c0, ev_c1; float last_conv_ms;
    float* h_pin_ir; size_t pin_ir_cap;
    std::mutex conv_mu;
};

cudaError_t fs_wave_alloc(fs_ctx* ctx, fs_lane* lane, uint32_t cap, uint32_t max_depth);
void fs_wave_free(fs_wave_buffers* wb);
cudaError_t fs_wave_trace_batch(fs_ctx* ctx, fs_lane* lane, const fs_trace_params& tp, unsigned long long* d_hist,
                                fs_path_dbg* d_dbg);
cudaError_t fs_wave_reset_counters(fs_ctx* ctx, int reset_overflow);
cudaError_t fs_wave_debug_rays(fs_ctx* ctx, const fs_trace_params& tp, const float* d_rays, const float* d_tmax,
                               uint64_t n, float* d_t, uint32_t* d_tri, uint8_t* d_hit);

cudaError_t fs_ir_build_multi(fs_ctx* ctx, const unsigned long long* d_hist, uint32_t s0, uint32_t n, uint64_t n_paths,
                              const fs_ptr_table& d_ir);
cudaError_t fs_conv_update_ir_multi(fs_ctx* ctx, uint32_t s0, uint32_t n, cudaStream_t st);
cudaError_t fs_ir_build_bands(fs_ctx* ctx, const unsigned long long* d_hist_src, uint64_t n_paths, uint64_t noise_seed,
                              float* d_ir_out);
cudaError_t fs_ir_build(fs_ctx* ctx, const unsigned long long* d_hist_src, uint64_t n_paths,
                        const float* d_energy_in, float* d_ir_out);

cudaError_t fs_conv_setup(fs_ctx* ctx);
void fs_conv_teardown(fs_ctx* ctx);
cudaError_t fs_conv_source_alloc(fs_ctx* ctx, uint32_t source, bool reset_history);
void fs_conv_source_free(fs_ctx* ctx, uint32_t source);
cudaError_t fs_conv_update_ir(fs_ctx* ctx, uint32_t source, cudaStream_t st);
cudaError_t fs_conv_run(fs_ctx* ctx, const uint32_t* sources, uint32_t n_src, const float* d_in, float* d_out, uint32_t n_blocks,
                        cudaStream_t st);
cudaError_t fs_conv_rfft(fs_ctx* ctx, const float* d_in, uint32_t n, float2* d_out, cudaStream_t st);
```

### audio-pathtracer_b200/csrc/fs_wavefront.cu

```cuda
#include "fs_internal.h"

namespace {

constexpr int WF_THREADS = 256;

#ifndef FS_STREAM_HINTS
#define FS_STREAM_HINTS 0
#endif
#if FS_STREAM_HINTS
#define FS_ST4(ptr, v) __stcs((ptr), (v))
#define FS_ST2(ptr, v) __stcs((ptr), (v))
#define FS_LD4(ptr) __ldcs(ptr)
#define FS_LD2(ptr) __ldcs(ptr)
#else
#define FS_ST4(ptr, v) (*(ptr) = (v))
#define FS_ST2(ptr, v) (*(ptr) = (v))
#define FS_LD4(ptr) (*(ptr))
#define FS_LD2(ptr) (*(ptr))
#endif

enum { MODE_BVH = 0, MODE_TOP = 1, MODE_BRUTE = 2 };

__device__ __forceinline__ uint32_t lane_id() { return threadIdx.x & 31u; }

// ... 965 lines not shown
        }
    }
    (void)guard;
    if (COUNT) flush_counters(dc, vc);
}


#ifndef FS_W8_SSTACK
#define FS_W8_SSTACK 6
#endif
#define FS_W8_STACK_SIZE 40
struct w8_stack {
    uint2* sh;
    uint2* loc;
    __device__ __forceinline__ void put(int i, uint2 e) const { if (i < FS_W8_SSTACK) sh[i * TR_THREADS] = e; else loc[i - FS_W8_SSTACK] = e; }
    __device__ __forceinline__ uint2 get(int i) const { return (i < FS_W8_SSTACK) ? sh[i * TR_THREADS] : loc[i - FS_W8_SSTACK]; }
};

__device__ __forceinline__ void tr_init8(tr_state& s, const fs_bvh_view& bv, fs_vec3 o, fs_vec3 d)
{
    s.o = o; s.d = d;
    const float dx = (fabsf(d.x) > 1e-30f) ? d.x : ((d.x < 0.0f) ? -1e-30f : 1e-30f);
    const float dy = (fabsf(d.y) > 1e-30f) ? d.y : ((d.y < 0.0f) ? -1e-30f : 1e-30f);
    const float dz = (fabsf(d.z) > 1e-30f) ? d.z : ((d.z < 0.0f) ? -1e-30f : 1e-30f);
    s.idx = fs_rcp_fast(dx); s.idy = fs_rcp_fast(dy); s.idz = fs_rcp_fast(dz);
    s.oodx = s.oody = s.oodz = 0.0f;
    s.oct = ((~__float_as_uint(s.idx)) >> 31) | (((~__float_as_uint(s.idy)) >> 31) << 1) | (((~__float_as_uint(s.idz)) >> 31) << 2);
    s.node = bv.n_tris ? 0 : TR_SENT; s.leaf = 0; s.sp = 0; s.tc = 0; s.te = 0;
}

#define FS_Q8(w, B) __uint_as_float(__byte_perm((w), magic, 0x7504u | ((B) << 4)))

__device__ __forceinline__ void w8_step(const fs_bvh_view& bv, tr_state& s, const w8_stack& stack, const float tlimit,
                                        uint32_t& hleaf, uint32_t& lmask, uint32_t& tri_base, uint32_t* overflow)
{
    const uint32_t magic = bv.w8_magic;
    const uint4* p = bv.w8nodes + (size_t)s.node * 5;
    const uint4 u0 = ldg_u4(p), u1 = ldg_u4(p + 1), u2 = ldg_u4(p + 2), u3 = ldg_u4(p + 3), u4 = ldg_u4(p + 4);
    const float ax = __uint_as_float(u0.w & 0x7f800000u) * s.idx, ay = __uint_as_float(u1.x) * s.idy, az = __uint_as_float(u1.y) * s.idz;
    const float bx = fmaf(-32768.0f, ax, (__uint_as_float(u0.x) - s.o.x) * s.idx);
    const float by = fmaf(-32768.0f, ay, (__uint_as_float(u0.y) - s.o.y) * s.idy);
    const float bz = fmaf(-32768.0f, az, (__uint_as_float(u0.z) - s.o.z) * s.idz);
    const bool px = (s.oct & 1u) != 0u, py = (s.oct & 2u) != 0u, pz = (s.oct & 4u) != 0u;
    const uint32_t nx0 = px ? u2.x : u3.z, nx1 = px ? u2.y : u3.w, fx0 = px ? u3.z : u2.x, fx1 = px ? u3.w : u2.y;
    const uint32_t ny0 = py ? u2.z : u4.x, ny1 = py ? u2.w : u4.y, fy0 = py ? u4.x : u2.z, fy1 = py ? u4.y : u2.w;
    const uint32_t nz0 = pz ? u3.x : u4.z, nz1 = pz ? u3.y : u4.w, fz0 = pz ? u4.z : u3.x, fz1 = pz ? u4.w : u3.y;
    uint32_t H = 0u;
#define FS_W8_CHILD(J, W, B)                                                                                          \
    {                                                                                                                 \
        const float tn = fmaxf(fmaxf(fmaf(FS_Q8(nx##W, B), ax, bx), fmaf(FS_Q8(ny##W, B), ay, by)),                   \
                               fmaxf(fmaf(FS_Q8(nz##W, B), az, bz), 0.0f));                                           \
        const float tf = fminf(fminf(fmaf(FS_Q8(fx##W, B), ax, bx), fmaf(FS_Q8(fy##W, B), ay, by)),                   \
                               fminf(fmaf(FS_Q8(fz##W, B), az, bz), tlimit));                                         \
        if (tn <= tf) H |= 1u << (J);                                                                                 \
    }
    FS_W8_CHILD(0, 0, 0u) FS_W8_CHILD(1, 0, 1u) FS_W8_CHILD(2, 0, 2u) FS_W8_CHILD(3, 0, 3u)
    FS_W8_CHILD(4, 1, 0u) FS_W8_CHILD(5, 1, 1u) FS_W8_CHILD(6, 1, 2u) FS_W8_CHILD(7, 1, 3u)
#undef FS_W8_CHILD
    const uint32_t imask = u0.w & 0xffu;
    lmask = (u0.w >> 8) & 0xffu;
    hleaf = H & lmask;
    tri_base = u1.w;
    uint32_t P = H & imask;
    if (s.oct & 4u) P = ((P & 0x0fu) << 4) | (P >> 4);
    if (s.oct & 2u) P = ((P & 0x33u) << 2) | ((P >> 2) & 0x33u);
    if (s.oct & 1u) P = ((P & 0x55u) << 1) | ((P >> 1) & 0x55u);
    uint32_t gb = u1.z, gm = (P << 8) | imask;
    if (P == 0u) {
        if (s.sp == 0) { s.node = TR_SENT; return; }
        --s.sp;
        const uint2 e = stack.get(s.sp);
        gb = e.x; gm = e.y;
    }
    const uint32_t pbit = 31u - (uint32_t)__clz((int)gm);
    gm ^= 1u << pbit;
    const uint32_t slot = (pbit - 8u) ^ s.oct;
    s.node = (int)(gb + (uint32_t)__popc(gm & ((1u << slot) - 1u)));
    if (gm >> 8) {
        if (s.sp < FS_W8_STACK_SIZE) { stack.put(s.sp, make_uint2(gb, gm)); ++s.sp; } else *overflow = 1u;
    }
}

#define FS_TQ_CAP 160
#define TQ_INVALID 0xffffffffu
#define TQ_WARPS (TR_THREADS / 32)
#define TR_SMEM_TQ (FS_SSTACK * TR_THREADS * sizeof(int) + TR_THREADS * sizeof(unsigned long long) + \
                    TQ_WARPS * FS_TQ_CAP * sizeof(uint32_t) + TQ_WARPS * sizeof(uint32_t) + TR_THREADS * sizeof(uint32_t))

#ifndef FS_DRAIN_SPLIT
#define FS_DRAIN_SPLIT 1
#endif
#ifndef FS_PREFETCH_PUSHED
#define FS_PREFETCH_PUSHED 0
#endif
#ifndef FS_PREFETCH_TRIS
#define FS_PREFETCH_TRIS 0
#endif
#ifndef FS_TRI_TEX
#define FS_TRI_TEX 0
#endif
#define FS_TQ8_CAP 288
#define TR_SMEM_TQ8 (FS_W8_SSTACK * TR_THREADS * sizeof(uint2) + TR_THREADS * sizeof(unsigned long long) + \
                     TQ_WARPS * FS_TQ8_CAP * sizeof(uint32_t) + TQ_WARPS * sizeof(uint32_t) + TR_THREADS * sizeof(uint32_t))
template <bool COUNT, int TEX, bool ANY, bool W8>
__global__ void __launch_bounds__(TR_THREADS, FS_TR_MINBLOCKS)
k_trace_q(const fs_bvh_view bv, const float4* __restrict__ ray_o, const float4* __restrict__ ray_d,
          const uint32_t* __restrict__ count_ptr, uint32_t* __restrict__ cursor,
          float2* __restrict__ hits, uint32_t* __restrict__ conn_queue, uint32_t* __restrict__ conn_count,
          fs_path_dbg* __restrict__ dbg, fs_dev_counters* __restrict__ dc, const uint32_t REFILL_MIN,
          const uint32_t NODE_MIN, const uint32_t FLUSH_MIN)
{
    constexpr bool DRAIN_SPLIT = FS_DRAIN_SPLIT != 0;
    constexpr uint32_t QCAP = W8 ? FS_TQ8_CAP : FS_TQ_CAP;
    constexpr int SST = W8 ? FS_W8_SSTACK : FS_SSTACK;
    const uint32_t lane = lane_id(), warp = threadIdx.x >> 5;
    const uint32_t count = *count_ptr;
    extern __shared__ __align__(8) unsigned char smem_raw[];
    int* const sstack = reinterpret_cast<int*>(smem_raw);
    uint2* const gstack = reinterpret_cast<uint2*>(smem_raw);
    unsigned long long* const skey = reinterpret_cast<unsigned long long*>(smem_raw + (W8 ? FS_W8_SSTACK * sizeof(uint2) : FS_SSTACK * sizeof(int)) * TR_THREADS);
    uint32_t* const squeue = reinterpret_cast<uint32_t*>(skey + TR_THREADS) + warp * QCAP;
    uint32_t* const sqcount = reinterpret_cast<uint32_t*>(skey + TR_THREADS) + TQ_WARPS * QCAP + warp;
    uint32_t* const whelp = reinterpret_cast<uint32_t*>(skey + TR_THREADS) + TQ_WARPS * QCAP + TQ_WARPS + (threadIdx.x & ~31u);
    unsigned long long* const mykey = skey + threadIdx.x;
    unsigned long long* const wkey = skey + (threadIdx.x & ~31u);
    int lstack[W8 ? 1 : FS_STACK_SIZE - FS_SSTACK];
    uint2 lstack8[W8 ? FS_W8_STACK_SIZE - FS_W8_SSTACK : 1];
    tr_stack<false> stack; stack.sh = sstack + threadIdx.x; stack.loc = lstack;
    w8_stack stack8; stack8.sh = gstack + threadIdx.x; stack8.loc = lstack8;
    const float4* const tris = W8 ? bv.tris8 : bv.tris;
    const unsigned long long KEY_NONE = ((unsigned long long)0x7f800000u << 32) | 0xffffffffull;
    for (uint32_t i = lane; i < QCAP; i += 32) squeue[i] = TQ_INVALID;
    if (lane == 0) *sqcount = 0u;
    *mykey = KEY_NONE;
    whelp[lane] = 0u;
    uint32_t owner = lane;
    __syncwarp();
    tr_state s;
    s.node = TR_SENT; s.leaf = 0; s.sp = 0; s.tc = 0; s.te = 0;
    s.o = fs_mk(0.f, 0.f, 0.f); s.d = s.o; s.idx = s.idy = s.idz = s.oodx = s.oody = s.oodz = 0.f;
    bool running = false, exhausted = false;
    uint32_t j = 0;
    uint32_t* const ovf_p = &dc->overflow;
    float bt = __int_as_float(0x7f800000);
    uint32_t qn = 0;
    uint32_t ray_steps = 0;
    fs_visit_counters vc; vc.nodes = 0; vc.tris = 0;
    for (;;) {
        const uint32_t m_idle = __ballot_sync(FULLM, !running);
        if (!exhausted && ((uint32_t)__popc(m_idle) >= REFILL_MIN)) {
            const uint32_t n = (uint32_t)__popc(m_idle);
            uint32_t base = 0;
            if (lane == 0) base = atomicAdd(cursor, n);
            base = __shfl_sync(FULLM, base, 0);
            if (base + n >= count) exhausted = true;
            if (!running) {
                const uint32_t jj = base + (uint32_t)__popc(m_idle & ((1u << lane) - 1u));
                if (jj < count) {
                    const float4 a = FS_LD4(ray_o + jj), b = FS_LD4(ray_d + jj);
                    if (W8) tr_init8(s, bv, fs_mk(a.x, a.y, a.z), fs_mk(b.x, b.y, b.z));
                    else tr_init<true>(s, bv, fs_mk(a.x, a.y, a.z), fs_mk(b.x, b.y, b.z));
                    bt = ANY ? a.w : __int_as_float(0x7f800000); *mykey = KEY_NONE;
                    j = ANY ? __float_as_uint(b.w) : jj; running = true;
                    if (COUNT) ray_steps = 0;
                }
            }
        }
        if (!__any_sync(FULLM, running)) break;
        for (;;) {
            for (;;) {
                const bool can = running && s.node >= 0 && s.node != TR_SENT;
                const uint32_t m_can = __ballot_sync(FULLM, can);
                if (m_can == 0u || qn >= FLUSH_MIN) break;
                if (NODE_MIN && qn && (uint32_t)__popc(m_can) < NODE_MIN) break;
                uint32_t nl = 0;
                if (can) {
                    if (COUNT) { vc.nodes++; ray_steps++; }
                    if (W8) {
                        uint32_t hleaf, lmask, tri_base;
                        w8_step(bv, s, stack8, bt, hleaf, lmask, tri_base, ovf_p);
                        nl = (uint32_t)__popc(hleaf);
                        if (nl) {
                            uint32_t* q = squeue + atomicAdd(sqcount, nl);
                            const uint32_t e0 = (tri_base << 5) | owner;
                            do {
                                const uint32_t bit = hleaf & (0u - hleaf);
                                *q++ = e0 + ((uint32_t)__popc(lmask & (bit - 1u)) << 5);
                                hleaf ^= bit;
                            } while (hleaf);
                        }
                    } else {
                        const float INF = __int_as_float(0x7f800000);
                        float k0, k1, k2, k3; int v0, v1, v2, v3;
                        wide_children<2, TEX>(bv, s, bt, k0, k1, k2, k3, v0, v1, v2, v3);
                        const bool l0 = k0 != INF && v0 < 0, l1 = k1 != INF && v1 < 0, l2 = k2 != INF && v2 < 0, l3 = k3 != INF && v3 < 0;
                        nl = (uint32_t)l0 + (uint32_t)l1 + (uint32_t)l2 + (uint32_t)l3;
                        if (nl) {
                            uint32_t* q = squeue + atomicAdd(sqcount, nl);
                            const uint32_t lm4 = owner - 4u;
#if FS_PREFETCH_TRIS
#define FS_PF_TRI(v) asm volatile("prefetch.global.L2 [%0];" :: "l"(bv.tris + (size_t)((uint32_t)(~(v)) >> 3) * 4))
#else
#define FS_PF_TRI(v)
#endif
                            if (l0) { *q = (uint32_t)v0 * 0xfffffffcu + lm4; FS_PF_TRI(v0); }
                            q += l0;
                            if (l1) { *q = (uint32_t)v1 * 0xfffffffcu + lm4; FS_PF_TRI(v1); }
                            q += l1;
                            if (l2) { *q = (uint32_t)v2 * 0xfffffffcu + lm4; FS_PF_TRI(v2); }
                            q += l2;
                            if (l3) { *q = (uint32_t)v3 * 0xfffffffcu + lm4; FS_PF_TRI(v3); }
#undef FS_PF_TRI
                        }
                        k0 = l0 ? INF : k0; k1 = l1 ? INF : k1; k2 = l2 ? INF : k2; k3 = l3 ? INF : k3;
                        FS_CSWAP(k0, v0, k1, v1) FS_CSWAP(k2, v2, k3, v3) FS_CSWAP(k0, v0, k2, v2) FS_CSWAP(k1, v1, k3, v3) FS_CSWAP(k1, v1, k2, v2)
                        w4_advance(s, stack, k0, k1, k2, k3, v0, v1, v2, v3, ovf_p);
                    }
                }
                qn += __reduce_add_sync(FULLM, nl);
            }
            __syncwarp();
            const uint32_t total = qn;
            for (uint32_t base = 0; base < total; base += 32) {
                const uint32_t idx = base + lane;
                const uint32_t e = idx < total ? squeue[idx] : TQ_INVALID;
                const uint32_t eo = e & 31u;
                const float ox = __shfl_sync(FULLM, s.o.x, eo), oy = __shfl_sync(FULLM, s.o.y, eo), oz = __shfl_sync(FULLM, s.o.z, eo);
                const float dx = __shfl_sync(FULLM, s.d.x, eo), dy = __shfl_sync(FULLM, s.d.y, eo), dz = __shfl_sync(FULLM, s.d.z, eo);
                const float bto = __shfl_sync(FULLM, bt, eo);
                if (e != TQ_INVALID) {
                    const uint32_t tri = e >> 5;
                    const float4* tq = tris + (size_t)tri * 4;
#if FS_TRI_TEX
                    const bool ttex = TEX >= 2 && bv.tris_tex;
                    const float4 a = ttex ? tex1Dfetch<float4>((cudaTextureObject_t)bv.tris_tex, (int)(tri * 4u)) : fs_ldg4(tq);
                    const float4 b = (FS_TRI_TEX >= 2 && ttex) ? tex1Dfetch<float4>((cudaTextureObject_t)bv.tris_tex, (int)(tri * 4u + 1u)) : fs_ldg4(tq + 1);
                    const float4 c = fs_ldg4(tq + 2);
#else
                    const float4 a = fs_ldg4(tq), b = fs_ldg4(tq + 1), c = fs_ldg4(tq + 2);
#endif
                    if (COUNT) vc.tris++;
                    squeue[idx] = TQ_INVALID;
                    float t;
                    const bool hit = fs_intersect_tri(fs_mk(ox, oy, oz), fs_mk(dx, dy, dz), fs_mk(a.x, a.y, a.z), fs_mk(b.x, b.y, b.z),
                                                      fs_mk(c.x, c.y, c.z), t);
                    if (ANY) {
                        if (hit && t < bto) *(volatile unsigned long long*)(wkey + eo) = 0ull;
                    } else if (hit && t <= bto) {
                        const unsigned long long mine = ((unsigned long long)__float_as_uint(t) << 32) | tri;
                        unsigned long long old = *(volatile unsigned long long*)(wkey + eo);
                        for (;;) {
                            const float told = __uint_as_float((uint32_t)(old >> 32));
                            bool better = t < told;
                            if (t == told) {
                                const uint32_t otri = (uint32_t)old;
                                better = otri == 0xffffffffu ||
                                         __float_as_uint(fs_ldg4(tq + 3).x) < __float_as_uint(fs_ldg4(tris + (size_t)otri * 4 + 3).x);
                            }
                            if (!better) break;
                            const unsigned long long prev = atomicCAS(wkey + eo, old, mine);
                            if (prev == old) break;
                            old = prev;
                        }
                    }
                }
            }
            __syncwarp();
            if (lane == 0) *sqcount = 0u;
            qn = 0u;
            const unsigned long long kk = *(volatile unsigned long long*)(wkey + owner);
            if (ANY) { if (running && kk != KEY_NONE) { s.node = TR_SENT; s.sp = 0; } }
            else bt = __uint_as_float((uint32_t)(kk >> 32));
            __syncwarp();
            const bool fin = running && s.node == TR_SENT;
            if (fin && owner != lane) { atomicSub(whelp + owner, 1u); running = false; owner = lane; }
            __syncwarp();
            const bool retire = fin && running && *(volatile uint32_t*)(whelp + lane) == 0u;
            if (ANY) {
                const bool conn = retire && kk == KEY_NONE;
                const uint32_t mc = __ballot_sync(FULLM, conn);
                if (mc) {
                    uint32_t slot = 0;
                    if (lane == 0) slot = atomicAdd(conn_count, (uint32_t)__popc(mc));
                    slot = __shfl_sync(FULLM, slot, 0);
                    if (conn) {
                        conn_queue[slot + (uint32_t)__popc(mc & ((1u << lane) - 1u))] = j;
                        if (dbg) dbg[j].connected = 1u;
                    }
                }
                if (retire) running = false;
            } else if (retire) {
                uint32_t ht = (uint32_t)kk;
                if (W8 && ht != 0xffffffffu) ht = bv.tri8_map[ht];
                FS_ST2(hits + j, make_float2(bt, __int_as_float((int)ht)));
                running = false;
                if (COUNT) { atomicMax(&dc->max_steps, ray_steps); atomicAdd(&dc->steps_hist[ray_steps / 8u < 15u ? ray_steps / 8u : 15u], 1u); }
            }
            if (DRAIN_SPLIT && exhausted) {
                const uint32_t m_free = __ballot_sync(FULLM, !running);
                const bool give = running && s.node != TR_SENT && s.sp >= 1 && s.sp <= SST;
                const uint32_t m_give = __ballot_sync(FULLM, give);
                const uint32_t nf = (uint32_t)__popc(m_free), ng = (uint32_t)__popc(m_give);
                const uint32_t n = nf < ng ? nf : ng;
                if (n) {
                    const uint32_t lt = (1u << lane) - 1u;
                    const uint32_t rf = (uint32_t)__popc(m_free & lt), rg = (uint32_t)__popc(m_give & lt);
                    const bool take = !running && rf < n;
                    const uint32_t donor = take ? __fns(m_give, 0u, (int)rf + 1) : lane;
                    const int dsp = __shfl_sync(FULLM, s.sp, donor);
                    const float ox = __shfl_sync(FULLM, s.o.x, donor), oy = __shfl_sync(FULLM, s.o.y, donor), oz = __shfl_sync(FULLM, s.o.z, donor);
                    const float dx = __shfl_sync(FULLM, s.d.x, donor), dy = __shfl_sync(FULLM, s.d.y, donor), dz = __shfl_sync(FULLM, s.d.z, donor);
                    const float ix = __shfl_sync(FULLM, s.idx, donor), iy = __shfl_sync(FULLM, s.idy, donor), iz = __shfl_sync(FULLM, s.idz, donor);
                    const float px = __shfl_sync(FULLM, s.oodx, donor), py = __shfl_sync(FULLM, s.oody, donor), pz = __shfl_sync(FULLM, s.oodz, donor);
                    const float dbt = __shfl_sync(FULLM, bt, donor);
                    const uint32_t down = __shfl_sync(FULLM, owner, donor);
                    if (take) {
                        const int h = (dsp + 1) >> 1;
                        s.o = fs_mk(ox, oy, oz); s.d = fs_mk(dx, dy, dz);
                        s.idx = ix; s.idy = iy; s.idz = iz; s.oodx = px; s.oody = py; s.oodz = pz;
                        bt = dbt; owner = down;
                        if (W8) {
                            const uint2* src = gstack + (threadIdx.x & ~31u) + donor;
                            for (int i = 0; i < h; ++i) stack8.sh[i * TR_THREADS] = src[(dsp - h + i) * TR_THREADS];
                            s.oct = ((~__float_as_uint(ix)) >> 31) | (((~__float_as_uint(iy)) >> 31) << 1) | (((~__float_as_uint(iz)) >> 31) << 2);
                            s.sp = h - 1;
                            const uint2 e = stack8.sh[s.sp * TR_THREADS];
                            uint32_t gm = e.y;
                            const uint32_t pbit = 31u - (uint32_t)__clz((int)gm);
                            gm ^= 1u << pbit;
                            const uint32_t slot = (pbit - 8u) ^ s.oct;
                            s.node = (int)(e.x + (uint32_t)__popc(gm & ((1u << slot) - 1u)));
                            if (gm >> 8) { stack8.sh[s.sp * TR_THREADS] = make_uint2(e.x, gm); ++s.sp; }
                        } else {
                            const int* src = sstack + (threadIdx.x & ~31u) + donor;
                            for (int i = 0; i < h; ++i) stack.sh[i * TR_THREADS] = src[(dsp - h + i) * TR_THREADS];
                            s.sp = h;
                            s.node = stack.pop(s.sp, 0.f);
                        }
                        running = true;
                        atomicAdd(whelp + down, 1u);
                    }
                    __syncwarp();
                    if (give && rg < n) s.sp -= (s.sp + 1) >> 1;
                }
            }
            const uint32_t m_run = __ballot_sync(FULLM, running);
            if (m_run == 0u) break;
            if (!exhausted && 32u - (uint32_t)__popc(m_run) >= REFILL_MIN) break;
// ... 93 lines not shown
    uint32_t* const shq = w32 + TQ_WARPS * QCAP + TQ_WARPS + warp * (PQ_SQ_CAP * 3);
    uint32_t* const whelp = w32 + TQ_WARPS * QCAP + TQ_WARPS + TQ_WARPS * (PQ_SQ_CAP * 3) + (threadIdx.x & ~31u);
    constexpr bool SPLIT = PQ_DRAIN_SPLIT != 0 && !W8;
    uint32_t my_ray = 0;
    unsigned long long* const mykey = skey + threadIdx.x;
    unsigned long long* const wkey = skey + (threadIdx.x & ~31u);
    int lstack[W8 ? 1 : FS_STACK_SIZE - FS_SSTACK];
    uint2 lstack8[W8 ? FS_W8_STACK_SIZE - FS_W8_SSTACK : 1];
    tr_stack<false> stack; stack.sh = sstack + threadIdx.x; stack.loc = lstack;
    w8_stack stack8; stack8.sh = gstack + threadIdx.x; stack8.loc = lstack8;
    const float4* const tris = W8 ? bv.tris8 : bv.tris;
    const unsigned long long KEY_NONE = ((unsigned long long)0x7f800000u << 32) | 0xffffffffull;
    if (lane == 0) *sqcount = 0u;
    *mykey = KEY_NONE;
    whelp[lane] = 0u;
    uint32_t owner = lane;
    __syncwarp();
    tr_state s;
    s.node = TR_SENT; s.leaf = 0; s.sp = 0; s.tc = 0; s.te = 0;
    s.o = fs_mk(0.f, 0.f, 0.f); s.d = s.o; s.idx = s.idy = s.idz = s.oodx = s.oody = s.oodz = 0.f;
    bool running = false, ready = false;
    uint32_t ticket = PQ_NO_TICKET;
    uint32_t* const ovf_p = &g->error;
    float bt = __int_as_float(0x7f800000);
    uint32_t qn = 0, sn = 0, polls = 0;
    const uint32_t stride = 2u * wb.cap;
    for (;;) {
        const bool need = (PQ_AHEAD || !running) && ticket == PQ_NO_TICKET;
        const uint32_t m_need = __ballot_sync(FULLM, need);
        const uint32_t m_run0 = __ballot_sync(FULLM, running);
        if ((uint32_t)__popc(m_need) >= REFILL_MIN || (m_need && m_run0 == 0u)) {
            uint32_t base = 0;
            if (lane == 0) base = atomicAdd(&g->head, (uint32_t)__popc(m_need));
            base = __shfl_sync(FULLM, base, 0);
            if (need) ticket = base + (uint32_t)__popc(m_need & lt);
        }
        if ((PQ_AHEAD || !running) && !ready && ticket != PQ_NO_TICKET && ticket < log_cap && ld_cg_u32(log_flag + ticket) == epoch) ready = true;
        if (!running && ready) {
            const float4 a = ld_cg_f4(log_o + ticket), b = ld_cg_f4(log_d + ticket);
            if (W8) tr_init8(s, bv, fs_mk(a.x, a.y, a.z), fs_mk(b.x, b.y, b.z));
            else tr_init<true>(s, bv, fs_mk(a.x, a.y, a.z), fs_mk(b.x, b.y, b.z));
            bt = __int_as_float(0x7f800000); *mykey = KEY_NONE;
            my_ray = ticket;
            running = true; ticket = PQ_NO_TICKET; ready = false;
        }
        const uint32_t m_run = __ballot_sync(FULLM, running);
        if (m_run == 0u && sn == 0u) {
            const uint32_t dn = ld_cg_u32(&g->done);
            const uint32_t tl = ld_cg_u32(&g->tail);
            if (dn == tl || ld_cg_u32(&g->error)) break;
            if (++polls > (1u << 21)) { if (lane == 0) atomicMax(&g->error, 3u); break; }
            __nanosleep(PQ_IDLE_NS);
            continue;
        }
        if (m_run) {
            for (;;) {
                const bool can = running && s.node >= 0 && s.node != TR_SENT;
                const uint32_t m_can = __ballot_sync(FULLM, can);
                if (m_can == 0u || qn >= FLUSH_MIN) break;
                if (NODE_MIN && qn && (uint32_t)__popc(m_can) < NODE_MIN) break;
                uint32_t nl = 0;
                if (can) {
                    if (W8) {
                        uint32_t hleaf, lmask, tri_base;
                        w8_step(bv, s, stack8, bt, hleaf, lmask, tri_base, ovf_p);
                        nl = (uint32_t)__popc(hleaf);
                        if (nl) {
                            uint32_t* q = squeue + atomicAdd(sqcount, nl);
                            const uint32_t e0 = (tri_base << 5) | lane;
                            do {
                                const uint32_t bit = hleaf & (0u - hleaf);
                                *q++ = e0 + ((uint32_t)__popc(lmask & (bit - 1u)) << 5);
                                hleaf ^= bit;
                            } while (hleaf);
                        }
                    } else {
                        const float INF = __int_as_float(0x7f800000);
                        float k0, k1, k2, k3; int v0, v1, v2, v3;
                        wide_children<2, TEX>(bv, s, bt, k0, k1, k2, k3, v0, v1, v2, v3, stop, NTOP);
                        const bool l0 = k0 != INF && v0 < 0, l1 = k1 != INF && v1 < 0, l2 = k2 != INF && v2 < 0, l3 = k3 != INF && v3 < 0;
                        nl = (uint32_t)l0 + (uint32_t)l1 + (uint32_t)l2 + (uint32_t)l3;
                        if (nl) {
                            uint32_t* q = squeue + atomicAdd(sqcount, nl);
                            const uint32_t lm4 = owner - 4u;
                            if (l0) *q = (uint32_t)v0 * 0xfffffffcu + lm4;
                            q += l0;
                            if (l1) *q = (uint32_t)v1 * 0xfffffffcu + lm4;
                            q += l1;
                            if (l2) *q = (uint32_t)v2 * 0xfffffffcu + lm4;
                            q += l2;
                            if (l3) *q = (uint32_t)v3 * 0xfffffffcu + lm4;
                        }
                        k0 = l0 ? INF : k0; k1 = l1 ? INF : k1; k2 = l2 ? INF : k2; k3 = l3 ? INF : k3;
                        FS_CSWAP(k0, v0, k1, v1) FS_CSWAP(k2, v2, k3, v3) FS_CSWAP(k0, v0, k2, v2) FS_CSWAP(k1, v1, k3, v3) FS_CSWAP(k1, v1, k2, v2)
                        w4_advance(s, stack, k0, k1, k2, k3, v0, v1, v2, v3, ovf_p);
                    }
                }
                qn += __reduce_add_sync(FULLM, nl);
            }
            __syncwarp();
            const uint32_t total = qn;
            for (uint32_t base = 0; base < total; base += 32) {
                const uint32_t idx = base + lane;
                const uint32_t e = idx < total ? squeue[idx] : TQ_INVALID;
                const uint32_t eo = e & 31u;
                const float ox = __shfl_sync(FULLM, s.o.x, eo), oy = __shfl_sync(FULLM, s.o.y, eo), oz = __shfl_sync(FULLM, s.o.z, eo);
                const float dx = __shfl_sync(FULLM, s.d.x, eo), dy = __shfl_sync(FULLM, s.d.y, eo), dz = __shfl_sync(FULLM, s.d.z, eo);
                const float bto = __shfl_sync(FULLM, bt, eo);
                if (e != TQ_INVALID) {
                    const uint32_t tri = e >> 5;
                    const float4* tq = tris + (size_t)tri * 4;
                    const float4 a = fs_ldg4(tq), b = fs_ldg4(tq + 1), c = fs_ldg4(tq + 2);
                    float t;
                    if (fs_intersect_tri(fs_mk(ox, oy, oz), fs_mk(dx, dy, dz), fs_mk(a.x, a.y, a.z), fs_mk(b.x, b.y, b.z), fs_mk(c.x, c.y, c.z), t)
                        && t <= bto) {
                        const unsigned long long mine = ((unsigned long long)__float_as_uint(t) << 32) | tri;
                        unsigned long long old = *(volatile unsigned long long*)(wkey + eo);
                        for (;;) {
                            const float told = __uint_as_float((uint32_t)(old >> 32));
                            bool better = t < told;
                            if (t == told) {
                                const uint32_t otri = (uint32_t)old;
                                better = otri == 0xffffffffu ||
                                         __float_as_uint(fs_ldg4(tq + 3).x) < __float_as_uint(fs_ldg4(tris + (size_t)otri * 4 + 3).x);
                            }
                            if (!better) break;
                            const unsigned long long prev = atomicCAS(wkey + eo, old, mine);
                            if (prev == old) break;
                            old = prev;
                        }
                    }
                }
            }
            __syncwarp();
            if (lane == 0) *sqcount = 0u;
            qn = 0u;
            const unsigned long long kk = *(volatile unsigned long long*)(wkey + owner);
            bt = __uint_as_float((uint32_t)(kk >> 32));
            __syncwarp();
            bool fin = running && s.node == TR_SENT;
            if (SPLIT) {
                if (fin && owner != lane) { atomicSub(whelp + owner, 1u); running = false; owner = lane; fin = false; }
                __syncwarp();
                fin = fin && *(volatile uint32_t*)(whelp + lane) == 0u;
            }
            const uint32_t m_fin = __ballot_sync(FULLM, fin);
            if (fin) {
                const uint32_t q = sn + (uint32_t)__popc(m_fin & lt);
                shq[0 * PQ_SQ_CAP + q] = my_ray;
                shq[1 * PQ_SQ_CAP + q] = __float_as_uint(bt);
                uint32_t ht = (uint32_t)kk;
                if (W8 && ht != 0xffffffffu) ht = bv.tri8_map[ht];
                shq[2 * PQ_SQ_CAP + q] = ht;
                running = false;
            }
            sn += (uint32_t)__popc(m_fin);
            if (SPLIT) {
                const bool idle = !running && !ready && ticket != PQ_NO_TICKET;
                const uint32_t m_free = __ballot_sync(FULLM, idle);
                const bool give = running && owner == lane && s.node != TR_SENT && s.sp >= 1 && s.sp <= FS_SSTACK;
                const uint32_t m_give = __ballot_sync(FULLM, give);
                const uint32_t nf = (uint32_t)__popc(m_free), ng = (uint32_t)__popc(m_give);
                const uint32_t n = nf < ng ? nf : ng;
                if (n) {
                    const uint32_t rf = (uint32_t)__popc(m_free & lt), rg = (uint32_t)__popc(m_give & lt);
                    const bool take = idle && rf < n;
                    const uint32_t donor = take ? __fns(m_give, 0u, (int)rf + 1) : lane;
                    const int dsp = __shfl_sync(FULLM, s.sp, donor);
                    const float ox = __shfl_sync(FULLM, s.o.x, donor), oy = __shfl_sync(FULLM, s.o.y, donor), oz = __shfl_sync(FULLM, s.o.z, donor);
                    const float dx = __shfl_sync(FULLM, s.d.x, donor), dy = __shfl_sync(FULLM, s.d.y, donor), dz = __shfl_sync(FULLM, s.d.z, donor);
                    const float ix = __shfl_sync(FULLM, s.idx, donor), iy = __shfl_sync(FULLM, s.idy, donor), iz = __shfl_sync(FULLM, s.idz, donor);
                    const float px = __shfl_sync(FULLM, s.oodx, donor), py = __shfl_sync(FULLM, s.oody, donor), pz = __shfl_sync(FULLM, s.oodz, donor);
                    const float dbt = __shfl_sync(FULLM, bt, donor);
                    if (take) {
                        const int h = (dsp + 1) >> 1;
                        const int* src = sstack + (threadIdx.x & ~31u) + donor;
                        for (int i = 0; i < h; ++i) stack.sh[i * TR_THREADS] = src[(dsp - h + i) * TR_THREADS];
                        s.o = fs_mk(ox, oy, oz); s.d = fs_mk(dx, dy, dz);
                        s.idx = ix; s.idy = iy; s.idz = iz; s.oodx = px; s.oody = py; s.oodz = pz;
                        s.sp = h; bt = dbt; owner = donor;
                        s.node = stack.pop(s.sp, 0.f);
                        running = true;
                        atomicAdd(whelp + donor, 1u);
                    }
                    __syncwarp();
                    if (give && rg < n) s.sp -= (s.sp + 1) >> 1;
                }
            }
        }
        if (sn >= PQ_SHADE_MIN || (sn && (uint32_t)__popc(__ballot_sync(FULLM, running)) < (PQ_TAIL_LANES ? PQ_TAIL_LANES : 1u))) {
            __syncwarp();
            for (uint32_t base = 0; base < sn; base += 32) {
                const uint32_t qi = base + lane;
                bool emit = false;
                fs_vec3 pos = fs_mk(0.f, 0.f, 0.f), dir = pos;
                float prob = 1.0f; uint32_t spk_out = 0;
                if (qi < sn) {
                    const uint32_t ri = shq[0 * PQ_SQ_CAP + qi];
                    const float4 ra = ld_cg_f4(log_o + ri), rb = ld_cg_f4(log_d + ri);
                    const uint32_t spk = __float_as_uint(ra.w);
                    const uint32_t sp_id = spk & 0x3fffffu, k = (spk >> 22) + 1u;
                    const float t = __uint_as_float(shq[1 * PQ_SQ_CAP + qi]);
                    const int tri = (int)shq[2 * PQ_SQ_CAP + qi];
                    const fs_vec3 o = fs_mk(ra.x, ra.y, ra.z);
                    const fs_vec3 d = fs_mk(rb.x, rb.y, rb.z);
                    const float pdf_in = rb.w;
                    fs_vec3 nrm = fs_mk(0.f, 0.f, 0.f);
                    bool cont = true, hit = false;
                    uint32_t nodes = k, mat = 0;
                    float seg = 0.f;
                    if (tri < 0) {
                        if (!tp.lobes) wb.end_pos[sp_id] = make_float4(o.x, o.y, o.z, __uint_as_float(k));
                        else if (k >= 2u) {
                            float4* rp = wb.rec + (size_t)(k - 1u) * stride + sp_id;
                            float4 rv = ld_cg_f4(rp);
// ... 443 lines not shown
    const size_t smem = (MODE == MODE_TOP) ? (size_t)tp.n_top * 64 : 0;
    const int occ_ext = resident_ctas(k_extend<COUNT, MODE>, WF_THREADS, smem);
    const int occ_con = resident_ctas(k_connect<COUNT, MODE>, WF_THREADS, smem);
    if (smem > 48 * 1024) {
        cudaFuncSetAttribute(k_extend<COUNT, MODE>, cudaFuncAttributeMaxDynamicSharedMemorySize, (int)smem);
        cudaFuncSetAttribute(k_connect<COUNT, MODE>, cudaFuncAttributeMaxDynamicSharedMemorySize, (int)smem);
    }
    const bool timing = (tp.flags & FS_FLAG_TIME_KERNELS) != 0;
    cudaEvent_t* ev = nullptr;
    if (timing) {
        if (ctx->kev.size() < ctx->kev_used + 4) {
            size_t old = ctx->kev.size();
            ctx->kev.resize(ctx->kev_used + 4);
            for (size_t i = old; i < ctx->kev.size(); ++i) cudaEventCreate(&ctx->kev[i]);
        }
        ev = &ctx->kev[ctx->kev_used];
        ctx->kev_used += 4;
    }
    const uint32_t nq = tp.max_depth + 4;
    k_reset_queues<<<(nq + 63) / 64, 64, 0, st>>>(wb.q_count, wb.q_cursor, nq, ctx->d_counters, 0);
    ctx->launches.fetch_add(1);
    const uint32_t warps_needed = (2u * tp.batch + 31u) / 32u;
    uint32_t grid_ext = (uint32_t)(ctx->sm_count * occ_ext);
    uint32_t ctas_needed = (warps_needed + WF_THREADS / 32 - 1) / (WF_THREADS / 32);
    if (grid_ext > ctas_needed) grid_ext = ctas_needed ? ctas_needed : 1;
    if (timing) cudaEventRecord(ev[0], st);
    if (tp.max_depth == 0) {
        k_init_ends<<<(2u * tp.batch + 255u) / 256u, 256, 0, st>>>(tp, wb);
        ctx->launches.fetch_add(1);
    }
    for (uint32_t k = 0; k < tp.max_depth; ++k) {
        k_extend<COUNT, MODE><<<grid_ext, WF_THREADS, smem, st>>>(tp, wb, k, (int)(k & 1u), ctx->d_counters);
        ctx->launches.fetch_add(1);
        ++ctx->stats.extend_launches;
    }
    if (timing) cudaEventRecord(ev[1], st);
    uint32_t grid_con = (uint32_t)(ctx->sm_count * occ_con);
    uint32_t ctas_con = ((tp.batch + 31u) / 32u + WF_THREADS / 32 - 1) / (WF_THREADS / 32);
    if (grid_con > ctas_con) grid_con = ctas_con ? ctas_con : 1;
    k_connect<COUNT, MODE><<<grid_con, WF_THREADS, smem, st>>>(tp, wb, ctx->d_counters, d_dbg);
    ctx->launches.fetch_add(1);
    if (timing) cudaEventRecord(ev[2], st);
    uint32_t grid_ev = (uint32_t)ctx->sm_count * 8u;
    const uint32_t ctas_ev = (tp.batch / 4u + WF_THREADS / 32 - 1) / (WF_THREADS / 32) + 1;
    if (grid_ev > ctas_ev) grid_ev = ctas_ev;
    k_eval<false><<<grid_ev, WF_THREADS, 0, st>>>(tp, wb, d_hist, ctx->d_counters, d_dbg);
    ctx->launches.fetch_add(1);
    if (timing) cudaEventRecord(ev[3], st);
    return cudaGetLastError();
}


template <bool COUNT>
static cudaError_t launch_batch_split(fs_ctx* ctx, fs_lane* lane, const fs_trace_params& tp, unsigned long long* d_hist,
                                      fs_path_dbg* d_dbg)
{
    cudaStream_t st = lane->stream;
    fs_wave_buffers& wb = lane->wb;
    int* occ = ctx->occ + (COUNT ? 4 : 0);
    if (!occ[0]) occ[0] = resident_ctas(k_trace_closest<COUNT, 2, true>, TR_THREADS, TR_SMEM_CLOSEST);
    if (!occ[1]) occ[1] = resident_ctas(k_trace_q<COUNT, 2, false, false>, TR_THREADS, TR_SMEM_TQ);
    if (!occ[3]) occ[3] = resident_ctas(k_trace_q<COUNT, 0, false, true>, TR_THREADS, TR_SMEM_TQ8);
    if (!occ[2]) occ[2] = resident_ctas(k_trace_any<COUNT, 2, true>, TR_THREADS, TR_SMEM_ANY);
    const bool use_w8 = ctx->tune_tq && tp.bv.w8nodes != nullptr;
    const int occ_tr = occ[0], occ_tq = use_w8 ? occ[3] : occ[1], occ_any = occ[2];
    const bool timing = (tp.flags & FS_FLAG_TIME_KERNELS) != 0;
    cudaEvent_t* ev = nullptr;
    if (timing) {
        if (ctx->kev.size() < ctx->kev_used + 4) {
            size_t old = ctx->kev.size();
            ctx->kev.resize(ctx->kev_used + 4);
            for (size_t i = old; i < ctx->kev.size(); ++i) cudaEventCreate(&ctx->kev[i]);
        }
        ev = &ctx->kev[ctx->kev_used];
        ctx->kev_used += 4;
    }
    const uint32_t nq = tp.max_depth + 4;
    k_reset_queues<<<(nq + 63) / 64, 64, 0, st>>>(wb.q_count, wb.q_cursor, nq, ctx->d_counters, 0);
    ctx->launches.fetch_add(1);
    const uint32_t D = tp.max_depth;
    const uint32_t n_sub = 2u * tp.batch;
    uint32_t grid_sh = (n_sub + FS_SG_THREADS - 1) / FS_SG_THREADS;
    if (grid_sh > (uint32_t)ctx->sm_count * (2048u / FS_SG_THREADS)) grid_sh = (uint32_t)ctx->sm_count * (2048u / FS_SG_THREADS);
    const bool use_tq = (ctx->tune_tq && tp.bv.wnodes != nullptr && ctx->bvh.max_leaf == 1) || use_w8;
    uint32_t grid_tr = (uint32_t)(ctx->sm_count * (use_tq ? occ_tq : occ_tr));
    const uint32_t ctas_needed = (n_sub + TR_THREADS - 1) / TR_THREADS;
    if (grid_tr > ctas_needed) grid_tr = ctas_needed ? ctas_needed : 1;
    if (timing) cudaEventRecord(ev[0], st);
    if (D == 0) {
        k_init_ends<<<(n_sub + 255u) / 256u, 256, 0, st>>>(tp, wb);
        ctx->launches.fetch_add(1);
    } else {
        const bool mega_ok = ctx->tune_mega == 1u || (ctx->tune_mega == 2u && tp.batch >= FS_MEGA_MIN_BATCH && tp.bv.n_tris >= 4096u &&
                                                      ctx->conv_active.load() == 0);
        const bool mega = !COUNT && use_tq && wb.log_o && mega_ok && (uint64_t)n_sub * D <= wb.log_cap;
        const uint32_t k0 = mega ? (ctx->tune_mega_from < D ? ctx->tune_mega_from : D) : D;
        for (uint32_t k = 0; k <= D; ++k) {
            k_shade_gen<<<grid_sh, FS_SG_THREADS, 0, st>>>(tp, wb, k, ctx->d_counters);
            ctx->launches.fetch_add(1);
            if (k == D) break;
            if (k == k0) {
                const bool texq = tp.bv.wnodes_tex && ctx->tune_tex >= 2;
                int& occ_pq = ctx->occ[use_w8 ? 10 : (texq ? 8 : 9)];
                if (!occ_pq) occ_pq = use_w8 ? resident_ctas(k_path_q<0, true>, TR_THREADS, PQ_SMEM8)
                                             : (texq ? resident_ctas(k_path_q<2, false>, TR_THREADS, PQ_SMEM) : resident_ctas(k_path_q<0, false>, TR_THREADS, PQ_SMEM));
                const uint32_t epoch = ++wb.pq_epoch;
                pq_globals* g = (pq_globals*)wb.pq;
                k_pq_seed<<<ctx->sm_count * 4, 256, 0, st>>>(wb, wb.log_o, wb.log_d, wb.log_flag, epoch, g, k0);
                uint32_t grid_pq = (uint32_t)(ctx->sm_count * occ_pq) / (ctx->cur_lanes ? ctx->cur_lanes : 1u);
                if (grid_pq > ctas_needed) grid_pq = ctas_needed ? ctas_needed : 1;
                cudaEvent_t* te = nullptr;
                if (timing) {
                    if (ctx->tev.size() < ctx->tev_used + 2) {
                        size_t old = ctx->tev.size();
                        ctx->tev.resize(ctx->tev_used + 2);
                        for (size_t i = old; i < ctx->tev.size(); ++i) cudaEventCreate(&ctx->tev[i]);
                    }
                    te = &ctx->tev[ctx->tev_used];
                    ctx->tev_used += 2;
                    cudaEventRecord(te[0], st);
                }
                if (use_w8) k_path_q<0, true><<<grid_pq, TR_THREADS, PQ_SMEM8, st>>>(tp, wb, wb.log_o, wb.log_d, wb.log_flag, epoch, wb.log_cap, g,
                                                                                   ctx->tune_refill, ctx->tune_tq_node_min, ctx->tune_tq_flush);
                else if (texq) k_path_q<2, false><<<grid_pq, TR_THREADS, PQ_SMEM, st>>>(tp, wb, wb.log_o, wb.log_d, wb.log_flag, epoch, wb.log_cap, g,
                                                                          ctx->tune_refill, ctx->tune_tq_node_min, ctx->tune_tq_flush);
                else k_path_q<0, false><<<grid_pq, TR_THREADS, PQ_SMEM, st>>>(tp, wb, wb.log_o, wb.log_d, wb.log_flag, epoch, wb.log_cap, g,
                                                                     ctx->tune_refill, ctx->tune_tq_node_min, ctx->tune_tq_flush);
                if (timing) cudaEventRecord(te[1], st);
                ctx->stats.persistent_launches += 1;
                k_pq_finish<<<1, 1, 0, st>>>(wb, g, D, ctx->d_counters, k0);
                ctx->launches.fetch_add(3);
                ctx->stats.extend_launches += 1;
                break;
            }
            const bool wide = tp.bv.wnodes != nullptr;
            const int texm = (wide ? tp.bv.wnodes_tex : tp.bv.nodes_tex) ? (int)ctx->tune_tex : 0;
            cudaEvent_t* te = nullptr;
            if (timing) {
                if (ctx->tev.size() < ctx->tev_used + 2) {
                    size_t old = ctx->tev.size();
                    ctx->tev.resize(ctx->tev_used + 2);
                    for (size_t i = old; i < ctx->tev.size(); ++i) cudaEventCreate(&ctx->tev[i]);
                }
                te = &ctx->tev[ctx->tev_used];
                ctx->tev_used += 2;
                cudaEventRecord(te[0], st);
            }
#define FS_LAUNCH_TRACE(TEXV, WIDEV)                                                                                   \
            k_trace_closest<COUNT, TEXV, WIDEV><<<grid_tr, TR_THREADS, TR_SMEM_CLOSEST, st>>>(tp.bv, wb.st_pos[k & 1u], wb.st_nrm[k & 1u], \
                wb.q_count + k, wb.q_cursor + k, wb.hit, ctx->d_counters, ctx->tune_refill, ctx->tune_node_min, ctx->tune_tri_min)
#define FS_LAUNCH_TQ(TEXV, W8V)                                                                                        \
            k_trace_q<COUNT, TEXV, false, W8V><<<grid_tr, TR_THREADS, W8V ? TR_SMEM_TQ8 : TR_SMEM_TQ, st>>>(tp.bv, wb.st_pos[k & 1u], \
                wb.st_nrm[k & 1u], wb.q_count + k, wb.q_cursor + k, wb.hit, nullptr, nullptr, nullptr, ctx->d_counters, ctx->tune_refill, \
                ctx->tune_tq_node_min, ctx->tune_tq_flush)
            if (use_w8) FS_LAUNCH_TQ(0, true);
            else if (use_tq) { if (texm >= 2) FS_LAUNCH_TQ(2, false); else FS_LAUNCH_TQ(0, false); }
            else if (wide) { if (texm >= 2) FS_LAUNCH_TRACE(2, true); else FS_LAUNCH_TRACE(0, true); }
            else { if (texm >= 2) FS_LAUNCH_TRACE(2, false); else FS_LAUNCH_TRACE(0, false); }
#undef FS_LAUNCH_TQ
#undef FS_LAUNCH_TRACE
            if (timing) cudaEventRecord(te[1], st);
            ctx->launches.fetch_add(1);
            ++ctx->stats.extend_launches;
        }
    }
    if (timing) cudaEventRecord(ev[1], st);
    uint32_t grid_cg = (tp.batch + WF_THREADS - 1) / WF_THREADS;
// ... 17 lines not shown
    const uint32_t ctas_any = (tp.batch + TR_THREADS - 1) / TR_THREADS;
    if (!all && grid_any > ctas_any) grid_any = ctas_any ? ctas_any : 1;
    const float4* any_o = all ? wb.all_o : wb.st_pos[0];
    const float4* any_d = all ? wb.all_d : wb.st_nrm[0];
    uint32_t* any_conn = all ? wb.all_conn : wb.conn_queue;
    {
        const bool wide = tp.bv.wnodes != nullptr;
        const bool tex = (wide ? tp.bv.wnodes_tex : tp.bv.nodes_tex) && ctx->tune_tex;
#define FS_LAUNCH_ANY(TEXV, WIDEV)                                                                                     \
        k_trace_any<COUNT, TEXV, WIDEV><<<grid_any, TR_THREADS, TR_SMEM_ANY, st>>>(tp.bv, any_o, any_d, wb.q_count + (D + 2), \
            wb.q_cursor + (D + 2), any_conn, wb.q_count + (D + 1), ctx->d_counters, all ? nullptr : d_dbg, ctx->tune_refill, ctx->tune_node_min)
#define FS_LAUNCH_ANYQ(TEXV, W8V)                                                                                      \
        k_trace_q<COUNT, TEXV, true, W8V><<<grid_any, TR_THREADS, W8V ? TR_SMEM_TQ8 : TR_SMEM_TQ, st>>>(tp.bv, any_o, any_d,       \
            wb.q_count + (D + 2), wb.q_cursor + (D + 2), nullptr, any_conn, wb.q_count + (D + 1), all ? nullptr : d_dbg, ctx->d_counters, \
            ctx->tune_refill, ctx->tune_tq_node_min, ctx->tune_tq_flush)
        if (use_w8 && ctx->tune_tq >= 2) FS_LAUNCH_ANYQ(0, true);
        else if (use_tq && ctx->tune_tq >= 2) { if (tex) FS_LAUNCH_ANYQ(2, false); else FS_LAUNCH_ANYQ(0, false); }
        else if (wide) { if (tex) FS_LAUNCH_ANY(2, true); else FS_LAUNCH_ANY(0, true); }
        else { if (tex) FS_LAUNCH_ANY(2, false); else FS_LAUNCH_ANY(0, false); }
#undef FS_LAUNCH_ANYQ
#undef FS_LAUNCH_ANY
    }
    ctx->launches.fetch_add(2);
    if (timing) cudaEventRecord(ev[2], st);
    uint32_t grid_ev = (uint32_t)ctx->sm_count * 8u;
    const uint32_t ctas_ev = (tp.batch / 4u + WF_THREADS / 32 - 1) / (WF_THREADS / 32) + 1;
    if (!all && grid_ev > ctas_ev) grid_ev = ctas_ev;
    if (tp.flags & FS_FLAG_MIS) k_eval_mis<<<grid_ev, WF_THREADS, 0, st>>>(tp, wb, d_hist, ctx->d_counters);
    else if (all) k_eval<true><<<grid_ev, WF_THREADS, 0, st>>>(tp, wb, d_hist, ctx->d_counters, nullptr);
    else k_eval<false><<<grid_ev, WF_THREADS, 0, st>>>(tp, wb, d_hist, ctx->d_counters, d_dbg);
    ctx->launches.fetch_add(1);
    if (timing) cudaEventRecord(ev[3], st);
    return cudaGetLastError();
}

cudaError_t fs_wave_trace_batch(fs_ctx* ctx, fs_lane* lane, const fs_trace_params& tp, unsigned long long* d_hist,
                                fs_path_dbg* d_dbg)
{
    const bool count = (tp.flags & FS_FLAG_COUNT_VISITS) != 0;
    if (!(tp.flags & (FS_FLAG_FUSED_EXTEND | FS_FLAG_BRUTE_FORCE)))
        return count ? launch_batch_split<true>(ctx, lane, tp, d_hist, d_dbg) : launch_batch_split<false>(ctx, lane, tp, d_hist, d_dbg);
    switch (pick_mode(tp)) {
    case MODE_BRUTE: return launch_batch<false, MODE_BRUTE>(ctx, lane, tp, d_hist, d_dbg);
    case MODE_TOP:
        return count ? launch_batch<true, MODE_TOP>(ctx, lane, tp, d_hist, d_dbg)
                     : launch_batch<false, MODE_TOP>(ctx, lane, tp, d_hist, d_dbg);
    default:
        return count ? launch_batch<true, MODE_BVH>(ctx, lane, tp, d_hist, d_dbg)
                     : launch_batch<false, MODE_BVH>(ctx, lane, tp, d_hist, d_dbg);
    }
}

cudaError_t fs_wave_reset_counters(fs_ctx* ctx, int reset_overflow)
{
    k_reset_queues<<<1, 64, 0, ctx->stream>>>(nullptr, nullptr, 0, ctx->d_counters, reset_overflow ? 3 : 1);
    ctx->launches.fetch_add(1);
    return cudaGetLastError();
}

cudaError_t fs_wave_debug_rays(fs_ctx* ctx, const fs_trace_params& tp, const float* d_rays, const float* d_tmax,
                               uint64_t n, float* d_t, uint32_t* d_tri, uint8_t* d_hit)
{
    cudaStream_t st = ctx->stream;
    const int mode = pick_mode(tp);
    if (!(tp.flags & (FS_FLAG_FUSED_EXTEND | FS_FLAG_BRUTE_FORCE)) && n < 0xffffffffull) {
        float4 *ro = nullptr, *rd = nullptr; float2* hits = nullptr; uint32_t *misc = nullptr, *conn = nullptr;
        cudaError_t e;
        if ((e = cudaMalloc(&ro, sizeof(float4) * n)) != cudaSuccess) return e;
        if ((e = cudaMalloc(&rd, sizeof(float4) * n)) != cudaSuccess) { cudaFree(ro); return e; }
        if ((e = cudaMalloc(&hits, sizeof(float2) * n)) != cudaSuccess) { cudaFree(ro); cudaFree(rd); return e; }
        if ((e = cudaMalloc(&conn, 4 * n)) != cudaSuccess) { cudaFree(ro); cudaFree(rd); cudaFree(hits); return e; }
        if ((e = cudaMalloc(&misc, 4 * 4)) != cudaSuccess) { cudaFree(ro); cudaFree(rd); cudaFree(hits); cudaFree(conn); return e; }
        cudaMemsetAsync(misc, 0, 16, st);
        const uint32_t g = (uint32_t)((n + 255) / 256);
        k_dbg_pack<<<g, 256, 0, st>>>(d_rays, d_hit ? d_tmax : nullptr, n, ro, rd, misc, d_hit);
        const bool wide = tp.bv.wnodes != nullptr;
        const bool tex = (wide ? tp.bv.wnodes_tex : tp.bv.nodes_tex) && ctx->tune_tex;
        uint32_t grid = (uint32_t)((n + TR_THREADS - 1) / TR_THREADS);
        if (grid > (uint32_t)ctx->sm_count * 5u) grid = (uint32_t)ctx->sm_count * 5u;
        if (d_hit) {
#define FS_DBG_ANY(TEXV, WIDEV) k_trace_any<false, TEXV, WIDEV><<<grid, TR_THREADS, TR_SMEM_ANY, st>>>(tp.bv, ro, rd, misc, misc + 1, conn, misc + 2, ctx->d_counters, nullptr, ctx->tune_refill, ctx->tune_node_min)
#define FS_DBG_ANYQ(TEXV, W8V) k_trace_q<false, TEXV, true, W8V><<<grid, TR_THREADS, W8V ? TR_SMEM_TQ8 : TR_SMEM_TQ, st>>>(tp.bv, ro, rd, misc, misc + 1, nullptr, conn, misc + 2, nullptr, ctx->d_counters, ctx->tune_refill, ctx->tune_tq_node_min, ctx->tune_tq_flush)
            if (tp.bv.w8nodes && ctx->tune_tq >= 2) FS_DBG_ANYQ(0, true);
            else if (wide && ctx->tune_tq >= 2 && ctx->bvh.max_leaf == 1) { if (tex) FS_DBG_ANYQ(2, false); else FS_DBG_ANYQ(0, false); }
            else if (wide) { if (tex) FS_DBG_ANY(2, true); else FS_DBG_ANY(0, true); } else { if (tex) FS_DBG_ANY(2, false); else FS_DBG_ANY(0, false); }
#undef FS_DBG_ANYQ
#undef FS_DBG_ANY
            k_dbg_unpack_any<<<g, 256, 0, st>>>(conn, misc + 2, d_hit);
        } else {
#define FS_DBG_CL(TEXV, WIDEV) k_trace_closest<false, TEXV, WIDEV><<<grid, TR_THREADS, TR_SMEM_CLOSEST, st>>>(tp.bv, ro, rd, misc, misc + 1, hits, ctx->d_counters, ctx->tune_refill, ctx->tune_node_min, ctx->tune_tri_min)
#define FS_DBG_TQ(TEXV, W8V) k_trace_q<false, TEXV, false, W8V><<<grid, TR_THREADS, W8V ? TR_SMEM_TQ8 : TR_SMEM_TQ, st>>>(tp.bv, ro, rd, misc, misc + 1, hits, nullptr, nullptr, nullptr, ctx->d_counters, ctx->tune_refill, ctx->tune_tq_node_min, ctx->tune_tq_flush)
            if (tp.bv.w8nodes && ctx->tune_tq) FS_DBG_TQ(0, true);
            else if (wide && ctx->tune_tq && ctx->bvh.max_leaf == 1) { if (tex) FS_DBG_TQ(2, false); else FS_DBG_TQ(0, false); }
            else if (wide) { if (tex) FS_DBG_CL(2, true); else FS_DBG_CL(0, true); } else { if (tex) FS_DBG_CL(2, false); else FS_DBG_CL(0, false); }
#undef FS_DBG_TQ
#undef FS_DBG_CL
            k_dbg_unpack_closest<<<g, 256, 0, st>>>(tp.bv, hits, n, d_t, d_tri);
        }
        ctx->launches.fetch_add(3);
        e = cudaStreamSynchronize(st);
        cudaFree(ro); cudaFree(rd); cudaFree(hits); cudaFree(conn); cudaFree(misc);
        return e != cudaSuccess ? e : cudaGetLastError();
    }
    const size_t smem = (mode == MODE_TOP) ? (size_t)tp.n_top * 64 : 0;
    uint32_t grid = (uint32_t)((n + WF_THREADS - 1) / WF_THREADS);
    if (grid > (uint32_t)ctx->sm_count * 8u) grid = (uint32_t)ctx->sm_count * 8u;
    if (!grid) grid = 1;
    if (mode == MODE_BRUTE) k_debug_rays<MODE_BRUTE><<<grid, WF_THREADS, 0, st>>>(tp, d_rays, d_tmax, n, d_t, d_tri, d_hit, ctx->d_counters);
    else if (mode == MODE_TOP) {
        if (smem > 48 * 1024) cudaFuncSetAttribute(k_debug_rays<MODE_TOP>, cudaFuncAttributeMaxDynamicSharedMemorySize, (int)smem);
        k_debug_rays<MODE_TOP><<<grid, WF_THREADS, smem, st>>>(tp, d_rays, d_tmax, n, d_t, d_tri, d_hit, ctx->d_counters);
    } else k_debug_rays<MODE_BVH><<<grid, WF_THREADS, 0, st>>>(tp, d_rays, d_tmax, n, d_t, d_tri, d_hit, ctx->d_counters);
    ctx->launches.fetch_add(1);
    return cudaGetLastError();
}
```

Before: 261.5 million.

## Allow multi-triangle leaves in 4-wide BVH collapse with SAH leaf cost

Extends the 4-wide DP collapse so a subtree can become a single leaf of up to four triangles when its SAH leaf cost beats further splitting. To support this, the BVH2 triangles are reordered depth-first so each subtree covers a contiguous range. The treelet-queue traversal now expands a queued leaf entry into its triangles using a warp scan. The queue path is also enabled for any wide BVH under a triangle-count limit instead of only single-triangle leaves. The intent is fewer node visits and shallower trees, at the cost of more triangle tests per leaf and extra build passes.

```diff
diff --git a/audio-pathtracer_b200/csrc/fs_api.cu b/audio-pathtracer_b200/csrc/fs_api.cu
--- a/audio-pathtracer_b200/csrc/fs_api.cu
+++ b/audio-pathtracer_b200/csrc/fs_api.cu
@@ -123,6 +123,9 @@
     if (const char* e3 = getenv("FS_TUNE_TEX")) ctx->tune_tex = (uint32_t)atoi(e3);
     if (const char* e1 = getenv("FS_TUNE_REFILL")) { int v = atoi(e1); if (v >= 1 && v <= 32) ctx->tune_refill = (uint32_t)v; }
     if (const char* e2 = getenv("FS_TUNE_LEAF_MAX")) { int v = atoi(e2); if (v >= 1 && v <= 8) ctx->tune_leaf_max = (uint32_t)v; }
+    ctx->tune_wide_leaf = FS_WIDE_LEAF_DEFAULT; ctx->tune_leaf_cost = FS_LEAF_COST_DEFAULT;
+    if (const char* e19 = getenv("FS_TUNE_WIDE_LEAF")) { int v = atoi(e19); if (v >= 1 && v <= FS_WIDE_LEAF_MAX) ctx->tune_wide_leaf = (uint32_t)v; }
+    if (const char* e20 = getenv("FS_TUNE_LEAF_COST")) { float v = (float)atof(e20); if (v > 0.0f && v < 1e3f) ctx->tune_leaf_cost = v; }
     dev_guard g(dev);
     int rc = FS_OK;
     do {
@@ -384,7 +387,8 @@
     }
     uint64_t bvh_launches = 0;
     CK(fs_bvh_build(ctx->stream, ctx->d_verts, ctx->d_tri_mat, ctx->n_tris, &ctx->bvh, &bvh_launches,
-                    ctx->tune_leaf_max, ctx->tune_builder, ctx->tune_collapse | (ctx->tune_w8 ? 4u : 0u)));
+                    ctx->tune_leaf_max, ctx->tune_builder, ctx->tune_collapse | (ctx->tune_w8 ? 4u : 0u), ctx->tune_wide_leaf,
+                    ctx->tune_leaf_cost));
     CK(cudaStreamSynchronize(ctx->stream));
     ctx->launches.fetch_add(bvh_launches);
     ctx->stats.bvh_nodes = ctx->bvh.n_inner;
diff --git a/audio-pathtracer_b200/csrc/fs_bvh.cuh b/audio-pathtracer_b200/csrc/fs_bvh.cuh
--- a/audio-pathtracer_b200/csrc/fs_bvh.cuh
+++ b/audio-pathtracer_b200/csrc/fs_bvh.cuh
@@ -4,6 +4,14 @@
 
 #define FS_STACK_SIZE 64
 #define FS_LEAF_MAX 4
+#define FS_WIDE_LEAF_MAX 4
+#ifndef FS_WIDE_LEAF_DEFAULT
+#define FS_WIDE_LEAF_DEFAULT 4
+#endif
+#ifndef FS_LEAF_COST_DEFAULT
+#define FS_LEAF_COST_DEFAULT 1.0f
+#endif
+static_assert(FS_WIDE_LEAF_DEFAULT >= 1 && FS_WIDE_LEAF_DEFAULT <= FS_WIDE_LEAF_MAX, "4-wide leaves hold 1 to 4 triangles");
 #define FS_TOP_FLAG 0x40000000
 
 #if defined(FS_TRAVERSAL_GUARD)
diff --git a/audio-pathtracer_b200/csrc/fs_bvh_build.cu b/audio-pathtracer_b200/csrc/fs_bvh_build.cu
--- a/audio-pathtracer_b200/csrc/fs_bvh_build.cu
+++ b/audio-pathtracer_b200/csrc/fs_bvh_build.cu
@@ -575,12 +575,22 @@
     if (c1 >= 0) parent[c1] = (int)i;
     if (i == 0) parent[0] = -1;
 }
+struct wide_leaf_opt { float ct; int L; const uint32_t* cnt; };
 template <int W>
-__device__ __forceinline__ float wide_t(const float* T, int ref, int j) { return ref >= 0 ? __ldcg(T + (size_t)ref * W + (j - 1)) : 0.0f; }
-__device__ __forceinline__ float w8_t(const float* T, int ref, int j) { return wide_t<8>(T, ref, j); }
+__device__ __forceinline__ float wide_t(const float* T, const cbox& c, int j, float ct)
+{
+    return c.ref >= 0 ? __ldcg(T + (size_t)c.ref * W + (j - 1)) : ct * cbox_area(c);
+}
+__device__ __forceinline__ float wide_leaf_cost(const wide_leaf_opt& o, int n, const cbox& a, const cbox& b)
+{
+    if (o.L <= 1 || n == 0) return 3.0e38f;
+    const uint32_t c = __ldg(o.cnt + n);
+    const float dx = fmaxf(a.hx, b.hx) - fminf(a.lx, b.lx), dy = fmaxf(a.hy, b.hy) - fminf(a.ly, b.ly), dz = fmaxf(a.hz, b.hz) - fminf(a.lz, b.lz);
+    return c <= (uint32_t)o.L ? o.ct * (float)c * (dx * dy + dy * dz + dz * dx) : 3.0e38f;
+}
 template <int W>
 __global__ void k_wide_dp(uint32_t n_inner, const float4* __restrict__ nodes, const int* __restrict__ parent,
-                        const uint32_t* __restrict__ need, uint32_t* __restrict__ arrive, float* T)
+                        const uint32_t* __restrict__ need, uint32_t* __restrict__ arrive, float* T, const wide_leaf_opt lo)
 {
     const uint32_t i = blockIdx.x * blockDim.x + threadIdx.x;
     if (i >= n_inner || need[i] != 0u) return;
@@ -589,13 +599,13 @@
         cbox a, b;
         load_children(nodes, n, a, b);
         float ta[W], tb[W], t[W];
-        for (int j = 1; j <= W; ++j) { ta[j - 1] = wide_t<W>(T, a.ref, j); tb[j - 1] = wide_t<W>(T, b.ref, j); }
+        for (int j = 1; j <= W; ++j) { ta[j - 1] = wide_t<W>(T, a, j, lo.ct); tb[j - 1] = wide_t<W>(T, b, j, lo.ct); }
         cbox u;
         u.lx = fminf(a.lx, b.lx); u.hx = fmaxf(a.hx, b.hx); u.ly = fminf(a.ly, b.ly); u.hy = fmaxf(a.hy, b.hy);
         u.lz = fminf(a.lz, b.lz); u.hz = fmaxf(a.hz, b.hz);
         float best = 3.0e38f;
         for (int x = 1; x <= W - 1; ++x) best = fminf(best, ta[x - 1] + tb[W - 1 - x]);
-        t[0] = cbox_area(u) + best;
+        t[0] = fminf(cbox_area(u) + best, wide_leaf_cost(lo, n, a, b));
         for (int j = 2; j <= W; ++j) {
             float m = t[j - 2];
             for (int x = 1; x < j; ++x) m = fminf(m, ta[x - 1] + tb[j - x - 1]);
@@ -610,42 +620,128 @@
     }
 }
 
+__device__ __forceinline__ int subtree_leaf_ref(const float4* __restrict__ nodes, int n, uint32_t cnt)
+{
+    int r = n;
+    while (r >= 0) r = __float_as_int(nodes[(size_t)r * 4 + 3].x);
+    return ~(int)(((uint32_t)~r & ~7u) | (cnt - 1u));
+}
+
 template <int W>
-__device__ __forceinline__ int dp_cut(const float4* __restrict__ nodes, const float* __restrict__ T, int i, cbox* c)
+__device__ __forceinline__ int dp_cut(const float4* __restrict__ nodes, const float* __restrict__ T, int i, cbox* c, const wide_leaf_opt lo)
 {
     cbox st[W]; int sb[W]; int sp = 0, k = 0;
     {
         cbox l, r;
         load_children(nodes, i, l, r);
         float best = 3.0e38f; int ba = 1;
-        for (int x = 1; x <= W - 1; ++x) { const float v = wide_t<W>(T, l.ref, x) + wide_t<W>(T, r.ref, W - x); if (v < best) { best = v; ba = x; } }
+        for (int x = 1; x <= W - 1; ++x) { const float v = wide_t<W>(T, l, x, lo.ct) + wide_t<W>(T, r, W - x, lo.ct); if (v < best) { best = v; ba = x; } }
         st[0] = l; sb[0] = ba; st[1] = r; sb[1] = W - ba; sp = 2;
     }
     while (sp) {
         --sp;
         const cbox m = st[sp]; const int j = sb[sp];
-        if (m.ref < 0 || j == 1) { c[k++] = m; continue; }
+        if (m.ref < 0 || (j == 1 && lo.L <= 1)) { c[k++] = m; continue; }
         cbox x, y;
         load_children(nodes, m.ref, x, y);
-        float best = wide_t<W>(T, m.ref, 1); int ba = 0;
-        for (int q = 1; q < j; ++q) { const float v = wide_t<W>(T, x.ref, q) + wide_t<W>(T, y.ref, j - q); if (v < best) { best = v; ba = q; } }
-        if (!ba) { c[k++] = m; continue; }
+        const float t1 = wide_t<W>(T, m, 1, lo.ct);
+        float best = t1; int ba = 0;
+        for (int q = 1; q < j; ++q) { const float v = wide_t<W>(T, x, q, lo.ct) + wide_t<W>(T, y, j - q, lo.ct); if (v < best) { best = v; ba = q; } }
+        if (!ba) {
+            c[k] = m;
+            if (t1 == wide_leaf_cost(lo, m.ref, x, y)) c[k].ref = subtree_leaf_ref(nodes, m.ref, __ldg(lo.cnt + m.ref));
+            ++k;
+            continue;
+        }
         st[sp] = x; sb[sp] = ba; st[sp + 1] = y; sb[sp + 1] = j - ba; sp += 2;
     }
     return k;
 }
 
 __global__ void k_emit4_dp(uint32_t n_inner, const float4* __restrict__ nodes, const float* __restrict__ T, const float* __restrict__ grid,
-                           uint4* __restrict__ wnodes, int* __restrict__ wsrc)
+                           uint4* __restrict__ wnodes, int* __restrict__ wsrc, const wide_leaf_opt lo)
 {
     const uint32_t i = blockIdx.x * blockDim.x + threadIdx.x;
     if (i >= n_inner) return;
     const uint4 EMPTY = make_uint4(0x0000ffffu, 0x0000ffffu, 0x0000ffffu, 0x7fffffffu);
     cbox c[4];
-    const int k = dp_cut<4>(nodes, T, (int)i, c);
+    const int k = dp_cut<4>(nodes, T, (int)i, c, lo);
     for (int j = 0; j < 4; ++j) {
         wnodes[(size_t)i * 4 + j] = (j < k) ? quant_box(c[j].lx, c[j].hx, c[j].ly, c[j].hy, c[j].lz, c[j].hz, c[j].ref, grid) : EMPTY;
         wsrc[(size_t)i * 4 + j] = (j < k) ? c[j].src : -1;
+    }
+}
+
+__global__ void k_wide_leaf_stats(uint32_t n_slots, const uint4* __restrict__ wnodes, uint32_t* __restrict__ stats)
+{
+    const uint32_t s = blockIdx.x * blockDim.x + threadIdx.x;
+    if (s >= n_slots) return;
+    const int r = (int)wnodes[s].w;
+    if (r >= 0) return;
+    const uint32_t c = ((uint32_t)~r & 7u) + 1u;
+    atomicAdd(stats, 1u); atomicAdd(stats + 1, c); atomicMax(stats + 2, c);
+}
+
+__device__ __forceinline__ uint32_t ref_cnt(const uint32_t* cnt, int r) { return r >= 0 ? __ldcg(cnt + r) : ((uint32_t)~r & 7u) + 1u; }
+
+__global__ void k_subtree_cnt(uint32_t n_inner, const float4* __restrict__ nodes, const int* __restrict__ parent,
+                              const uint32_t* __restrict__ need, uint32_t* __restrict__ arrive, uint32_t* cnt)
+{
+    const uint32_t i = blockIdx.x * blockDim.x + threadIdx.x;
+    if (i >= n_inner || need[i] != 0u) return;
+    int n = (int)i;
+    for (;;) {
+        const float4 n3 = nodes[(size_t)n * 4 + 3];
+        __stcg(cnt + n, ref_cnt(cnt, __float_as_int(n3.x)) + ref_cnt(cnt, __float_as_int(n3.y)));
+        __threadfence();
+        const int p = parent[n];
+        if (p < 0) break;
+        if (atomicAdd(arrive + p, 1u) + 1u < need[p]) break;
+        __threadfence();
+        n = p;
+    }
+}
+
+__global__ void k_dfs_order(uint32_t n_inner, const float4* __restrict__ nodes, const int* __restrict__ parent,
+                            const uint32_t* __restrict__ cnt, int2* __restrict__ nref, uint32_t* __restrict__ src)
+{
+    const uint32_t i = blockIdx.x * blockDim.x + threadIdx.x;
+    if (i >= n_inner) return;
+    uint32_t first = 0;
+    for (int c = (int)i, p = parent[i]; p >= 0; c = p, p = parent[p]) {
+        const int l = __float_as_int(nodes[(size_t)p * 4 + 3].x);
+        if (l != c) first += ref_cnt(cnt, l);
+    }
+    const float4 n3 = nodes[(size_t)i * 4 + 3];
+    int r[2] = {__float_as_int(n3.x), __float_as_int(n3.y)};
+    for (int s = 0; s < 2; ++s) {
+        const uint32_t k = ref_cnt(cnt, r[s]);
+        if (r[s] < 0) {
+            const uint32_t old = (uint32_t)~r[s] >> 3;
+            for (uint32_t q = 0; q < k; ++q) src[first + q] = old + q;
+            r[s] = ~(int)((first << 3) | (k - 1u));
+        }
+        first += k;
+    }
+    nref[i] = make_int2(r[0], r[1]);
+}
+
+__global__ void k_dfs_apply(uint32_t n, uint32_t n_inner, const uint32_t* __restrict__ src, const int2* __restrict__ nref,
+                            const float4* __restrict__ tris, const uint32_t* __restrict__ tri_orig, const uint32_t* __restrict__ tri_mat,
+                            const float4* __restrict__ tri_nm, float4* __restrict__ tris_o, uint32_t* __restrict__ tri_orig_o,
+                            uint32_t* __restrict__ tri_mat_o, float4* __restrict__ tri_nm_o, float4* __restrict__ nodes)
+{
+    const uint32_t j = blockIdx.x * blockDim.x + threadIdx.x;
+    if (j < n) {
+        const uint32_t o = src[j];
+        for (int a = 0; a < 4; ++a) tris_o[(size_t)j * 4 + a] = tris[(size_t)o * 4 + a];
+        tri_orig_o[j] = tri_orig[o]; tri_mat_o[j] = tri_mat[o]; tri_nm_o[j] = tri_nm[o];
+    }
+    if (j < n_inner) {
+        const int2 r = nref[j];
+        float4 w = nodes[(size_t)j * 4 + 3];
+        w.x = __int_as_float(r.x); w.y = __int_as_float(r.y);
+        nodes[(size_t)j * 4 + 3] = w;
     }
 }
 
@@ -657,7 +753,7 @@
     cbox c[8];
     int k = 2;
     if (T) {
-        k = dp_cut<8>(nodes, T, (int)i, c);
+        k = dp_cut<8>(nodes, T, (int)i, c, wide_leaf_opt{0.0f, 1, nullptr});
     } else {
         load_children(nodes, (int)i, c[0], c[1]);
         while (k < 8) {
@@ -1326,6 +1422,74 @@
     return err;
 }
 
+static cudaError_t subtree_counts(cudaStream_t st, uint32_t n_inner, const float4* nodes, int* parent, uint32_t* need,
+                                  uint32_t* arrive, uint32_t* cnt, uint64_t* launches)
+{
+    const int TPB = 256;
+    const uint32_t g = (n_inner + TPB - 1) / TPB;
+    const cudaError_t err = cudaMemsetAsync(arrive, 0, 4ull * n_inner, st);
+    if (err != cudaSuccess) return err;
+    k_w8_parents<<<g, TPB, 0, st>>>(n_inner, nodes, parent, need);
+    k_subtree_cnt<<<g, TPB, 0, st>>>(n_inner, nodes, parent, need, arrive, cnt);
+    *launches += 2;
+    return cudaGetLastError();
+}
+
+static cudaError_t dfs_relayout(cudaStream_t st, uint32_t n, uint32_t n_inner, fs_bvh_device* out, const int* parent,
+                                const uint32_t* cnt, uint64_t* launches)
+{
+    cudaError_t err = cudaSuccess;
+    int2* nref = nullptr; uint32_t* src = nullptr;
+    float4 *tris = nullptr, *tri_nm = nullptr; uint32_t *tri_orig = nullptr, *tri_mat = nullptr;
+    const int TPB = 256;
+    BCHECK(cudaMalloc(&nref, sizeof(int2) * n_inner)); BCHECK(cudaMalloc(&src, 4ull * n));
+    BCHECK(cudaMalloc(&tris, sizeof(float4) * 4ull * n)); BCHECK(cudaMalloc(&tri_nm, sizeof(float4) * (size_t)n));
+    BCHECK(cudaMalloc(&tri_orig, 4ull * n)); BCHECK(cudaMalloc(&tri_mat, 4ull * n));
+    k_dfs_order<<<(n_inner + TPB - 1) / TPB, TPB, 0, st>>>(n_inner, out->nodes, parent, cnt, nref, src);
+    k_dfs_apply<<<(n + TPB - 1) / TPB, TPB, 0, st>>>(n, n_inner, src, nref, out->tris, out->tri_orig, out->tri_mat, out->tri_nm,
+                                                     tris, tri_orig, tri_mat, tri_nm, out->nodes);
+    *launches += 2;
+    BCHECK(cudaGetLastError());
+    BCHECK(cudaStreamSynchronize(st));
+    std::swap(out->tris, tris); std::swap(out->tri_orig, tri_orig); std::swap(out->tri_mat, tri_mat); std::swap(out->tri_nm, tri_nm);
+fail:
+    cudaFree(nref); cudaFree(src); cudaFree(tris); cudaFree(tri_nm); cudaFree(tri_orig); cudaFree(tri_mat);
+    return err;
+}
+
+static cudaError_t wide_dp_collapse(cudaStream_t st, uint32_t n, uint32_t n_inner, fs_bvh_device* out, const float* grid, int L,
+                                    float ct, uint64_t* launches, float* cost)
+{
+    cudaError_t err = cudaSuccess;
+    float* T4 = nullptr; int* par = nullptr; uint32_t *need = nullptr, *arr = nullptr, *cnt = nullptr;
+    const int TPB = 256;
+    const uint32_t g = (n_inner + TPB - 1) / TPB;
+    BCHECK(cudaMalloc(&T4, sizeof(float) * 4ull * n_inner)); BCHECK(cudaMalloc(&par, 4ull * n_inner));
+    BCHECK(cudaMalloc(&need, 4ull * n_inner)); BCHECK(cudaMalloc(&arr, 4ull * n_inner));
+    if (L > 1) {
+        BCHECK(cudaMalloc(&cnt, 4ull * n_inner));
+        BCHECK(subtree_counts(st, n_inner, out->nodes, par, need, arr, cnt, launches));
+        BCHECK(dfs_relayout(st, n, n_inner, out, par, cnt, launches));
+    }
+    {
+        const wide_leaf_opt run[3] = {{L > 1 ? ct : 0.0f, L, cnt}, {ct, L, cnt}, {ct, 1, nullptr}};
+        const int n_run = getenv("FS_VERBOSE") ? 3 : 1;
+        for (int r = 0; r < n_run; ++r) {
+            BCHECK(cudaMemsetAsync(arr, 0, 4ull * n_inner, st));
+            k_w8_parents<<<g, TPB, 0, st>>>(n_inner, out->nodes, par, need);
+            k_wide_dp<4><<<g, TPB, 0, st>>>(n_inner, out->nodes, par, need, arr, T4, run[r]);
+            *launches += 2;
+            if (r == 0) { k_emit4_dp<<<g, TPB, 0, st>>>(n_inner, out->nodes, T4, grid, out->wnodes, out->wsrc, run[r]); ++*launches; }
+            else BCHECK(cudaMemcpyAsync(cost + r - 1, T4, 4, cudaMemcpyDeviceToHost, st));
+        }
+    }
+    BCHECK(cudaGetLastError());
+    BCHECK(cudaStreamSynchronize(st));
+fail:
+    cudaFree(T4); cudaFree(par); cudaFree(need); cudaFree(arr); cudaFree(cnt);
+    return err;
+}
+
 static cudaError_t w8_build(cudaStream_t st, uint32_t n, uint32_t n_inner, const float4* nodes, const float4* tris,
                             fs_bvh_device* out, uint64_t* launches, bool dp)
 {
@@ -1354,7 +1518,7 @@
         BCHECK(cudaMalloc(&parent, 4ull * n_inner)); BCHECK(cudaMalloc(&need, 4ull * n_inner)); BCHECK(cudaMalloc(&arrive, 4ull * n_inner));
         BCHECK(cudaMemsetAsync(arrive, 0, 4ull * n_inner, st));
         k_w8_parents<<<(n_inner + TPB - 1) / TPB, TPB, 0, st>>>(n_inner, nodes, parent, need);
-        k_wide_dp<8><<<(n_inner + TPB - 1) / TPB, TPB, 0, st>>>(n_inner, nodes, parent, need, arrive, T);
+        k_wide_dp<8><<<(n_inner + TPB - 1) / TPB, TPB, 0, st>>>(n_inner, nodes, parent, need, arrive, T, wide_leaf_opt{0.0f, 1, nullptr});
         *launches += 2;
     }
     k_emit8<<<(n_inner + TPB - 1) / TPB, TPB, 0, st>>>(n_inner, nodes, T, tmp, ref); ++*launches;
@@ -1387,7 +1551,8 @@
 }
 
 cudaError_t fs_bvh_build(cudaStream_t st, const float* d_verts, const uint32_t* d_mats, uint64_t T64,
-                         fs_bvh_device* out, uint64_t* launches, uint32_t leaf_max_u, uint32_t builder, uint32_t collapse_u)
+                         fs_bvh_device* out, uint64_t* launches, uint32_t leaf_max_u, uint32_t builder, uint32_t collapse_u,
+                         uint32_t wide_leaf, float leaf_cost)
 {
     const int leaf_max = (int)(leaf_max_u < 1 ? 1 : (leaf_max_u > 8 ? 8 : leaf_max_u));
     const int collapse = (int)collapse_u;
@@ -1406,6 +1571,7 @@
     int *parent = nullptr, *queue = nullptr;
     const int TPB = 256;
     const uint32_t gb = (n + TPB - 1) / TPB;
+    float dp_cost[2] = {0.0f, 0.0f};
 
     BCHECK(cudaMalloc(&tlo, sizeof(float4) * n));
     BCHECK(cudaMalloc(&thi, sizeof(float4) * n));
@@ -1416,7 +1582,7 @@
     BCHECK(cudaMalloc(&vals0, 4ull * n));
     BCHECK(cudaMalloc(&vals1, 4ull * n));
     BCHECK(cudaMalloc(&block_hist, 4ull * 256 * n_blocks_sort));
-    BCHECK(cudaMalloc(&misc, 4 * 16));
+    BCHECK(cudaMalloc(&misc, 4 * 20));
     BCHECK(cudaMalloc(&arrive, 4ull * n_inner));
     BCHECK(cudaMalloc(&children, sizeof(int2) * n_inner));
     BCHECK(cudaMalloc(&ranges, sizeof(int2) * n_inner));
@@ -1433,7 +1599,7 @@
     BCHECK(cudaMalloc(&out->top_nodes, sizeof(float4) * 4ull * FS_TOP_CAP));
     out->n_inner = n_inner;
 
-    BCHECK(cudaMemsetAsync(misc, 0, 4 * 16, st));
+    BCHECK(cudaMemsetAsync(misc, 0, 4 * 20, st));
     BCHECK(cudaMemsetAsync(arrive, 0, 4ull * n_inner, st));
     k_init_bounds<<<1, 32, 0, st>>>(misc); ++*launches;
     k_tri_bounds<<<gb, TPB, 0, st>>>(d_verts, n, tlo, thi, misc, misc + 6); ++*launches;
@@ -1462,7 +1628,7 @@
         if (n < 4096) n_cand = 1;
         double best_cost = 0.0; int best = -1;
         float4* alt = nullptr; double* d_cost = nullptr;
-        float* cT4 = nullptr; int* cpar = nullptr; uint32_t *cneed = nullptr, *carr = nullptr;
+        float* cT4 = nullptr; int* cpar = nullptr; uint32_t *cneed = nullptr, *carr = nullptr, *ccnt = nullptr;
         if (n_cand > 1) { BCHECK(cudaMalloc(&alt, sizeof(float4) * 4ull * n_inner)); BCHECK(cudaMalloc(&d_cost, 8)); }
         for (int ci = 0; ci < n_cand; ++ci) {
             float4* dst = (n_cand > 1) ? alt : out->nodes;
@@ -1478,11 +1644,14 @@
                 if (!cT4) {
                     BCHECK(cudaMalloc(&cT4, sizeof(float) * 4ull * n_inner)); BCHECK(cudaMalloc(&cpar, 4ull * n_inner));
                     BCHECK(cudaMalloc(&cneed, 4ull * n_inner)); BCHECK(cudaMalloc(&carr, 4ull * n_inner));
+                    if (wide_leaf > 1) BCHECK(cudaMalloc(&ccnt, 4ull * n_inner));
                 }
                 float root_cost = 0.f;
+                if (wide_leaf > 1) BCHECK(subtree_counts(st, n_inner, dst, cpar, cneed, carr, ccnt, launches));
                 BCHECK(cudaMemsetAsync(carr, 0, 4ull * n_inner, st));
                 k_w8_parents<<<(n_inner + TPB - 1) / TPB, TPB, 0, st>>>(n_inner, dst, cpar, cneed);
-                k_wide_dp<4><<<(n_inner + TPB - 1) / TPB, TPB, 0, st>>>(n_inner, dst, cpar, cneed, carr, cT4);
+                k_wide_dp<4><<<(n_inner + TPB - 1) / TPB, TPB, 0, st>>>(n_inner, dst, cpar, cneed, carr, cT4,
+                                                                        wide_leaf_opt{wide_leaf > 1 ? leaf_cost : 0.0f, (int)wide_leaf, ccnt});
                 *launches += 2;
                 BCHECK(cudaMemcpyAsync(&root_cost, cT4, 4, cudaMemcpyDeviceToHost, st));
                 BCHECK(cudaStreamSynchronize(st));
@@ -1495,7 +1664,7 @@
             }
         }
         if (alt) { cudaStreamSynchronize(st); cudaFree(alt); cudaFree(d_cost); }
-        cudaFree(cT4); cudaFree(cpar); cudaFree(cneed); cudaFree(carr);
+        cudaFree(cT4); cudaFree(cpar); cudaFree(cneed); cudaFree(carr); cudaFree(ccnt);
         out->max_leaf = 1;
         {
             int sweeps = 0;
@@ -1527,19 +1696,7 @@
     }
     k_quant_grid<<<1, 32, 0, st>>>(out->nodes, grid); ++*launches;
     if ((collapse & 16) && n >= 3) {
-        float* T4 = nullptr; int* par = nullptr; uint32_t *need = nullptr, *arr = nullptr;
-        cudaError_t e4 = cudaSuccess;
-        if ((e4 = cudaMalloc(&T4, sizeof(float) * 4ull * n_inner)) == cudaSuccess && (e4 = cudaMalloc(&par, 4ull * n_inner)) == cudaSuccess &&
-            (e4 = cudaMalloc(&need, 4ull * n_inner)) == cudaSuccess && (e4 = cudaMalloc(&arr, 4ull * n_inner)) == cudaSuccess &&
-            (e4 = cudaMemsetAsync(arr, 0, 4ull * n_inner, st)) == cudaSuccess) {
-            k_w8_parents<<<(n_inner + TPB - 1) / TPB, TPB, 0, st>>>(n_inner, out->nodes, par, need);
-            k_wide_dp<4><<<(n_inner + TPB - 1) / TPB, TPB, 0, st>>>(n_inner, out->nodes, par, need, arr, T4);
-            k_emit4_dp<<<(n_inner + TPB - 1) / TPB, TPB, 0, st>>>(n_inner, out->nodes, T4, grid, out->wnodes, out->wsrc);
-            *launches += 3;
-            e4 = cudaStreamSynchronize(st);
-        }
-        cudaFree(T4); cudaFree(par); cudaFree(need); cudaFree(arr);
-        BCHECK(e4);
+        BCHECK(wide_dp_collapse(st, n, n_inner, out, grid, builder == 1 ? (int)wide_leaf : 1, leaf_cost, launches, dp_cost));
     } else {
         k_emit4<<<(n_inner + TPB - 1) / TPB, TPB, 0, st>>>(n_inner, out->nodes, grid, out->wnodes, out->wsrc, collapse & 1); ++*launches;
     }
@@ -1568,14 +1725,19 @@
         if (cudaCreateTextureObject(&out->wnodes_tex, &rd, &td, nullptr) != cudaSuccess) { out->wnodes_tex = 0; (void)cudaGetLastError(); }
     }
     k_top_treelet<<<1, 32, 0, st>>>(out->nodes, n_inner, FS_TOP_CAP, out->top_nodes, misc + 7, queue); ++*launches;
+    k_wide_leaf_stats<<<(4 * out->n_wide + TPB - 1) / TPB, TPB, 0, st>>>(4 * out->n_wide, out->wnodes, misc + 16); ++*launches;
     BCHECK(cudaGetLastError());
     if (builder == 1 && n >= 3 && out->max_leaf == 1 && (collapse & 4)) BCHECK(w8_build(st, n, n_inner, out->nodes, out->tris, out, launches, !(collapse & 8)));
     {
-        uint32_t h[16];
+        uint32_t h[20];
         BCHECK(cudaMemcpyAsync(h, misc, sizeof(h), cudaMemcpyDeviceToHost, st));
         BCHECK(cudaStreamSynchronize(st));
         out->n_top = h[7];
         if (n > 1 && !(builder == 1 && n >= 3)) out->max_leaf = h[8] ? h[8] : 1;
+        if (builder == 1 && n >= 3) out->max_leaf = h[18] ? h[18] : 1;
+        if (getenv("FS_VERBOSE"))
+            fprintf(stderr, "[frequensee] 4-wide nodes: %u, %u leaf slots, %.3f triangles per leaf (at most %u); DP root cost %.6g (leaves <= %u), %.6g (single-triangle leaves), leaf cost %.3g\n",
+                    out->n_wide, h[16], h[16] ? (double)h[17] / h[16] : 0.0, h[18], (double)dp_cost[0], wide_leaf, (double)dp_cost[1], (double)leaf_cost);
         out->extent = ord2f(h[6]);
         float hg[6];
         BCHECK(cudaMemcpy(hg, grid, sizeof(hg), cudaMemcpyDeviceToHost));
diff --git a/audio-pathtracer_b200/csrc/fs_internal.h b/audio-pathtracer_b200/csrc/fs_internal.h
--- a/audio-pathtracer_b200/csrc/fs_internal.h
+++ b/audio-pathtracer_b200/csrc/fs_internal.h
@@ -45,7 +45,9 @@
 
 cudaError_t fs_bvh_build(cudaStream_t st, const float* d_verts, const uint32_t* d_mats, uint64_t n_tris,
                          fs_bvh_device* out, uint64_t* launches, uint32_t leaf_max, uint32_t builder ,
-                         uint32_t collapse );
+                         uint32_t collapse ,
+                         uint32_t wide_leaf ,
+                         float leaf_cost );
 void fs_bvh_free(fs_bvh_device* b);
 cudaError_t fs_bvh_refit(cudaStream_t st, const float* d_verts, fs_bvh_device* b, uint64_t* launches, float* cost_ratio);
 
@@ -149,7 +151,8 @@
     std::vector<cudaEvent_t> tev; size_t tev_used;
     int sm_count;
     int occ[16];
-    uint32_t tune_refill, tune_leaf_max, tune_tex, tune_builder, tune_wide, tune_node_min, tune_tri_min, tune_collapse, tune_l2pin_mb, tune_tq, tune_tq_node_min, tune_tq_flush, tune_mega, tune_mega_from, tune_mega_lanes, cur_lanes, tune_w8;
+    uint32_t tune_refill, tune_leaf_max, tune_tex, tune_builder, tune_wide, tune_node_min, tune_tri_min, tune_collapse, tune_l2pin_mb, tune_tq, tune_tq_node_min, tune_tq_flush, tune_mega, tune_mega_from, tune_mega_lanes, cur_lanes, tune_w8, tune_wide_leaf;
+    float tune_leaf_cost;
     float* d_energy;
     float* d_amp;
     float* d_amp_all; uint32_t amp_all_cap;
diff --git a/audio-pathtracer_b200/csrc/fs_wavefront.cu b/audio-pathtracer_b200/csrc/fs_wavefront.cu
--- a/audio-pathtracer_b200/csrc/fs_wavefront.cu
+++ b/audio-pathtracer_b200/csrc/fs_wavefront.cu
@@ -1071,6 +1071,7 @@
 }
 
 #define FS_TQ_CAP 160
+#define FS_TQ_MAX_TRIS (1u << 24)
 #define TQ_INVALID 0xffffffffu
 #define TQ_WARPS (TR_THREADS / 32)
 #define TR_SMEM_TQ (FS_SSTACK * TR_THREADS * sizeof(int) + TR_THREADS * sizeof(unsigned long long) + \
@@ -1081,9 +1082,6 @@
 #endif
 #ifndef FS_PREFETCH_PUSHED
 #define FS_PREFETCH_PUSHED 0
-#endif
-#ifndef FS_PREFETCH_TRIS
-#define FS_PREFETCH_TRIS 0
 #endif
 #ifndef FS_TRI_TEX
 #define FS_TRI_TEX 0
@@ -1091,6 +1089,33 @@
 #define FS_TQ8_CAP 288
 #define TR_SMEM_TQ8 (FS_W8_SSTACK * TR_THREADS * sizeof(uint2) + TR_THREADS * sizeof(unsigned long long) + \
                      TQ_WARPS * FS_TQ8_CAP * sizeof(uint32_t) + TQ_WARPS * sizeof(uint32_t) + TR_THREADS * sizeof(uint32_t))
+template <bool W8>
+__device__ __forceinline__ uint32_t tq_scan(uint32_t e, uint32_t lane, uint32_t& excl)
+{
+    const uint32_t c = e == TQ_INVALID ? 0u : (W8 ? 1u : ((e >> 5) & 7u) + 1u);
+    uint32_t incl = c;
+    for (uint32_t o = 1; o < 32u; o <<= 1) {
+        const uint32_t y = __shfl_up_sync(FULLM, incl, o);
+        if (lane >= o) incl += y;
+    }
+    excl = incl - c;
+    return __shfl_sync(FULLM, incl, 31);
+}
+template <bool W8>
+__device__ __forceinline__ bool tq_pick(uint32_t e, uint32_t excl, uint32_t ntri, uint32_t cb, uint32_t lane, uint32_t& eo,
+                                        uint32_t& tri)
+{
+    const bool valid = e != TQ_INVALID;
+    const uint32_t before = (uint32_t)__popc(__ballot_sync(FULLM, valid && excl < cb));
+    const uint32_t rel = excl - cb;
+    const uint32_t heads = __reduce_or_sync(FULLM, (valid && excl >= cb && rel < 32u) ? 1u << rel : 0u);
+    const uint32_t k = (before + (uint32_t)__popc(heads & (0xffffffffu >> (31u - lane))) - 1u) & 31u;
+    const uint32_t ek = __shfl_sync(FULLM, e, k), xk = __shfl_sync(FULLM, excl, k);
+    eo = ek & 31u;
+    tri = W8 ? (ek >> 5) : (ek >> 8) + (cb + lane - xk);
+    return cb + lane < ntri;
+}
+
 template <bool COUNT, int TEX, bool ANY, bool W8>
 __global__ void __launch_bounds__(TR_THREADS, FS_TR_MINBLOCKS)
 k_trace_q(const fs_bvh_view bv, const float4* __restrict__ ray_o, const float4* __restrict__ ray_d,
@@ -1186,20 +1211,14 @@
                         nl = (uint32_t)l0 + (uint32_t)l1 + (uint32_t)l2 + (uint32_t)l3;
                         if (nl) {
                             uint32_t* q = squeue + atomicAdd(sqcount, nl);
-                            const uint32_t lm4 = owner - 4u;
-#if FS_PREFETCH_TRIS
-#define FS_PF_TRI(v) asm volatile("prefetch.global.L2 [%0];" :: "l"(bv.tris + (size_t)((uint32_t)(~(v)) >> 3) * 4))
-#else
-#define FS_PF_TRI(v)
-#endif
-                            if (l0) { *q = (uint32_t)v0 * 0xfffffffcu + lm4; FS_PF_TRI(v0); }
+                            const uint32_t lm32 = owner - 32u;
+                            if (l0) *q = (uint32_t)v0 * 0xffffffe0u + lm32;
                             q += l0;
-                            if (l1) { *q = (uint32_t)v1 * 0xfffffffcu + lm4; FS_PF_TRI(v1); }
+                            if (l1) *q = (uint32_t)v1 * 0xffffffe0u + lm32;
                             q += l1;
-                            if (l2) { *q = (uint32_t)v2 * 0xfffffffcu + lm4; FS_PF_TRI(v2); }
+                            if (l2) *q = (uint32_t)v2 * 0xffffffe0u + lm32;
                             q += l2;
-                            if (l3) { *q = (uint32_t)v3 * 0xfffffffcu + lm4; FS_PF_TRI(v3); }
-#undef FS_PF_TRI
+                            if (l3) *q = (uint32_t)v3 * 0xffffffe0u + lm32;
                         }
                         k0 = l0 ? INF : k0; k1 = l1 ? INF : k1; k2 = l2 ? INF : k2; k3 = l3 ? INF : k3;
                         FS_CSWAP(k0, v0, k1, v1) FS_CSWAP(k2, v2, k3, v3) FS_CSWAP(k0, v0, k2, v2) FS_CSWAP(k1, v1, k3, v3) FS_CSWAP(k1, v1, k2, v2)
@@ -1213,12 +1232,16 @@
             for (uint32_t base = 0; base < total; base += 32) {
                 const uint32_t idx = base + lane;
                 const uint32_t e = idx < total ? squeue[idx] : TQ_INVALID;
-                const uint32_t eo = e & 31u;
+                if (idx < total) squeue[idx] = TQ_INVALID;
+                uint32_t excl;
+                const uint32_t ntri = tq_scan<W8>(e, lane, excl);
+              for (uint32_t cb = 0; cb < ntri; cb += 32) {
+                uint32_t eo, tri;
+                const bool act = tq_pick<W8>(e, excl, ntri, cb, lane, eo, tri);
                 const float ox = __shfl_sync(FULLM, s.o.x, eo), oy = __shfl_sync(FULLM, s.o.y, eo), oz = __shfl_sync(FULLM, s.o.z, eo);
                 const float dx = __shfl_sync(FULLM, s.d.x, eo), dy = __shfl_sync(FULLM, s.d.y, eo), dz = __shfl_sync(FULLM, s.d.z, eo);
                 const float bto = __shfl_sync(FULLM, bt, eo);
-                if (e != TQ_INVALID) {
-                    const uint32_t tri = e >> 5;
+                if (act) {
                     const float4* tq = tris + (size_t)tri * 4;
 #if FS_TRI_TEX
                     const bool ttex = TEX >= 2 && bv.tris_tex;
@@ -1229,7 +1252,6 @@
                     const float4 a = fs_ldg4(tq), b = fs_ldg4(tq + 1), c = fs_ldg4(tq + 2);
 #endif
                     if (COUNT) vc.tris++;
-                    squeue[idx] = TQ_INVALID;
                     float t;
                     const bool hit = fs_intersect_tri(fs_mk(ox, oy, oz), fs_mk(dx, dy, dz), fs_mk(a.x, a.y, a.z), fs_mk(b.x, b.y, b.z),
                                                       fs_mk(c.x, c.y, c.z), t);
@@ -1253,6 +1275,7 @@
                         }
                     }
                 }
+              }
             }
             __syncwarp();
             if (lane == 0) *sqcount = 0u;
@@ -1512,14 +1535,14 @@
                         nl = (uint32_t)l0 + (uint32_t)l1 + (uint32_t)l2 + (uint32_t)l3;
                         if (nl) {
                             uint32_t* q = squeue + atomicAdd(sqcount, nl);
-                            const uint32_t lm4 = owner - 4u;
-                            if (l0) *q = (uint32_t)v0 * 0xfffffffcu + lm4;
+                            const uint32_t lm32 = owner - 32u;
+                            if (l0) *q = (uint32_t)v0 * 0xffffffe0u + lm32;
                             q += l0;
-                            if (l1) *q = (uint32_t)v1 * 0xfffffffcu + lm4;
+                            if (l1) *q = (uint32_t)v1 * 0xffffffe0u + lm32;
                             q += l1;
-                            if (l2) *q = (uint32_t)v2 * 0xfffffffcu + lm4;
+                            if (l2) *q = (uint32_t)v2 * 0xffffffe0u + lm32;
                             q += l2;
-                            if (l3) *q = (uint32_t)v3 * 0xfffffffcu + lm4;
+                            if (l3) *q = (uint32_t)v3 * 0xffffffe0u + lm32;
                         }
                         k0 = l0 ? INF : k0; k1 = l1 ? INF : k1; k2 = l2 ? INF : k2; k3 = l3 ? INF : k3;
                         FS_CSWAP(k0, v0, k1, v1) FS_CSWAP(k2, v2, k3, v3) FS_CSWAP(k0, v0, k2, v2) FS_CSWAP(k1, v1, k3, v3) FS_CSWAP(k1, v1, k2, v2)
@@ -1533,12 +1556,15 @@
             for (uint32_t base = 0; base < total; base += 32) {
                 const uint32_t idx = base + lane;
                 const uint32_t e = idx < total ? squeue[idx] : TQ_INVALID;
-                const uint32_t eo = e & 31u;
+                uint32_t excl;
+                const uint32_t ntri = tq_scan<W8>(e, lane, excl);
+              for (uint32_t cb = 0; cb < ntri; cb += 32) {
+                uint32_t eo, tri;
+                const bool act = tq_pick<W8>(e, excl, ntri, cb, lane, eo, tri);
                 const float ox = __shfl_sync(FULLM, s.o.x, eo), oy = __shfl_sync(FULLM, s.o.y, eo), oz = __shfl_sync(FULLM, s.o.z, eo);
                 const float dx = __shfl_sync(FULLM, s.d.x, eo), dy = __shfl_sync(FULLM, s.d.y, eo), dz = __shfl_sync(FULLM, s.d.z, eo);
                 const float bto = __shfl_sync(FULLM, bt, eo);
-                if (e != TQ_INVALID) {
-                    const uint32_t tri = e >> 5;
+                if (act) {
                     const float4* tq = tris + (size_t)tri * 4;
                     const float4 a = fs_ldg4(tq), b = fs_ldg4(tq + 1), c = fs_ldg4(tq + 2);
                     float t;
@@ -1561,6 +1587,7 @@
                         }
                     }
                 }
+              }
             }
             __syncwarp();
             if (lane == 0) *sqcount = 0u;
@@ -2170,7 +2197,7 @@
     const uint32_t n_sub = 2u * tp.batch;
     uint32_t grid_sh = (n_sub + FS_SG_THREADS - 1) / FS_SG_THREADS;
     if (grid_sh > (uint32_t)ctx->sm_count * (2048u / FS_SG_THREADS)) grid_sh = (uint32_t)ctx->sm_count * (2048u / FS_SG_THREADS);
-    const bool use_tq = (ctx->tune_tq && tp.bv.wnodes != nullptr && ctx->bvh.max_leaf == 1) || use_w8;
+    const bool use_tq = (ctx->tune_tq && tp.bv.wnodes != nullptr && ctx->bvh.n_tris <= FS_TQ_MAX_TRIS) || use_w8;
     uint32_t grid_tr = (uint32_t)(ctx->sm_count * (use_tq ? occ_tq : occ_tr));
     const uint32_t ctas_needed = (n_sub + TR_THREADS - 1) / TR_THREADS;
     if (grid_tr > ctas_needed) grid_tr = ctas_needed ? ctas_needed : 1;
@@ -2354,7 +2381,7 @@
 #define FS_DBG_ANY(TEXV, WIDEV) k_trace_any<false, TEXV, WIDEV><<<grid, TR_THREADS, TR_SMEM_ANY, st>>>(tp.bv, ro, rd, misc, misc + 1, conn, misc + 2, ctx->d_counters, nullptr, ctx->tune_refill, ctx->tune_node_min)
 #define FS_DBG_ANYQ(TEXV, W8V) k_trace_q<false, TEXV, true, W8V><<<grid, TR_THREADS, W8V ? TR_SMEM_TQ8 : TR_SMEM_TQ, st>>>(tp.bv, ro, rd, misc, misc + 1, nullptr, conn, misc + 2, nullptr, ctx->d_counters, ctx->tune_refill, ctx->tune_tq_node_min, ctx->tune_tq_flush)
             if (tp.bv.w8nodes && ctx->tune_tq >= 2) FS_DBG_ANYQ(0, true);
-            else if (wide && ctx->tune_tq >= 2 && ctx->bvh.max_leaf == 1) { if (tex) FS_DBG_ANYQ(2, false); else FS_DBG_ANYQ(0, false); }
+            else if (wide && ctx->tune_tq >= 2 && ctx->bvh.n_tris <= FS_TQ_MAX_TRIS) { if (tex) FS_DBG_ANYQ(2, false); else FS_DBG_ANYQ(0, false); }
             else if (wide) { if (tex) FS_DBG_ANY(2, true); else FS_DBG_ANY(0, true); } else { if (tex) FS_DBG_ANY(2, false); else FS_DBG_ANY(0, false); }
 #undef FS_DBG_ANYQ
 #undef FS_DBG_ANY
@@ -2363,7 +2390,7 @@
 #define FS_DBG_CL(TEXV, WIDEV) k_trace_closest<false, TEXV, WIDEV><<<grid, TR_THREADS, TR_SMEM_CLOSEST, st>>>(tp.bv, ro, rd, misc, misc + 1, hits, ctx->d_counters, ctx->tune_refill, ctx->tune_node_min, ctx->tune_tri_min)
 #define FS_DBG_TQ(TEXV, W8V) k_trace_q<false, TEXV, false, W8V><<<grid, TR_THREADS, W8V ? TR_SMEM_TQ8 : TR_SMEM_TQ, st>>>(tp.bv, ro, rd, misc, misc + 1, hits, nullptr, nullptr, nullptr, ctx->d_counters, ctx->tune_refill, ctx->tune_tq_node_min, ctx->tune_tq_flush)
             if (tp.bv.w8nodes && ctx->tune_tq) FS_DBG_TQ(0, true);
-            else if (wide && ctx->tune_tq && ctx->bvh.max_leaf == 1) { if (tex) FS_DBG_TQ(2, false); else FS_DBG_TQ(0, false); }
+            else if (wide && ctx->tune_tq && ctx->bvh.n_tris <= FS_TQ_MAX_TRIS) { if (tex) FS_DBG_TQ(2, false); else FS_DBG_TQ(0, false); }
             else if (wide) { if (tex) FS_DBG_CL(2, true); else FS_DBG_CL(0, true); } else { if (tex) FS_DBG_CL(2, false); else FS_DBG_CL(0, false); }
 #undef FS_DBG_TQ
 #undef FS_DBG_CL
```

Result: slower. 249.1 million (median of 6 runs) (-4.8%).
